# meirbon/rfw-rs

Measured on AMD Instinct MI355X. Metric: Mrays/s (primary+shadow, 1spp), higher is better.
Workload: dtype f32

## Files before the change

rfw-rs_amd/csrc/api_frame.cpp:

```cpp
#include "api_internal.h"

using namespace rfwapi;

namespace rfwapi {
thread_local std::string g_create_error;
}
namespace rfwhip {
static EnvSwitches g_env;
const EnvSwitches& env_switches() { return g_env; }
void read_env_switches()
{
    EnvSwitches e;
    auto set = [](const char* name) { const char* v = getenv(name); return v != nullptr && std::strcmp(v, "0") != 0; };
    e.build_trace = set("RFW_BUILD_TRACE");
    e.no_forest = set("RFW_NO_FOREST");
    e.lbvh_fenced = set("RFW_LBVH_FENCED");
    e.p2p_data_cached = set("RFW_P2P_DATA_CACHED");
    e.p2p_flags_finegrained = set("RFW_P2P_FLAGS_FINEGRAINED");
    if (const char* v = getenv("RFW_PACKET_AUTO_MAX_TRIANGLES")) e.packet_auto_max_triangles = strtoull(v, nullptr, 10);
    if (const char* v = getenv("RFW_SPATIAL_SPLITS")) { e.has_spatial_splits = true; e.spatial_splits = (float)std::max(0.0, atof(v)); }
    if (const char* v = getenv("RFW_PACKET_TRACE")) e.packet_trace = std::max(0, atoi(v));
    static std::mutex mu;
    std::lock_guard<std::mutex> g(mu);
    g_env = e;
// ... 737 lines not shown
        I->release_deform();
        if (I->dn_chain) (void)hipEventDestroy(I->dn_chain);
        I->d_disp_state.release(); I->d_disp_hist.release();
        if (I->disp_chain) (void)hipEventDestroy(I->disp_chain);
        release_overlay(I);
        for (auto& ev : I->ring)
            if (ev) (void)hipEventDestroy(ev);
        if (I->ev_fork) (void)hipEventDestroy(I->ev_fork);
        for (int k = 0; k < kMaxSub; k++) {
            if (I->ev_join[k]) (void)hipEventDestroy(I->ev_join[k]);
            if (I->sub[k]) (void)hipStreamDestroy(I->sub[k]);
        }
        if (I->own_stream) (void)hipStreamDestroy(I->own_stream);
    }
    delete I;
}

const char* rfw_hip_last_error(void* inst)
{
    if (!inst) return g_create_error.c_str();
    return static_cast<Instance*>(inst)->err.c_str();
}


static int render_impl(Instance* I, const rfw_camera_view_3d* views, uint32_t k, bool samples = false, uint32_t mode = RFW_HIP_RENDER_DEFAULT)
{
    if (I->slots.empty()) return do_render(I, views, k, samples, mode);
    Instance* cur = slot_ptr(I, I->cur_slot);
    const bool same_image = (k == 1 || samples) && !I->restart && cur->sample_count > 0 && cur->have_last_view &&
                            std::memcmp(&cur->last_view, views, sizeof(*views)) == 0 && cur->rendered_version == I->scene_version &&
                            cur->render_mode == mode;
    if (!same_image) {
        I->cur_slot = (I->cur_slot + 1) % (uint32_t)(I->slots.size() + 1);
        cur = slot_ptr(I, I->cur_slot);
        cur->sample_count = 0;
    }
    I->restart = false;
    cur->rendered_version = I->scene_version;
    if (cur != I) {
        cur->max_path_length = I->max_path_length; cur->clamp_value = I->clamp_value; cur->flags = I->flags; cur->timing = I->timing;
        for (int c = 0; c < 3; c++) cur->sky[c] = I->sky[c];
        cur->ao_samples = I->ao_samples; cur->ao_radius = I->ao_radius;
        cur->denoise = I->denoise; cur->denoise_colour = I->denoise_colour; cur->denoise_form = I->denoise_form;
    }
    int rc = ensure_slot_tlas(I, cur);
    if (rc == RFW_HIP_OK) rc = do_render(cur, views, k, samples, mode);
    if (rc != RFW_HIP_OK && cur != I && !cur->err.empty()) I->err = cur->err;
    return rc;
}

int rfw_hip_render(void* inst, const rfw_mat4* view_2d, const rfw_camera_view_3d* view, uint32_t mode)
{
    LOCK(inst);
    if (!view) return fail(I, RFW_HIP_E_INVALID, "render: null view");
    CHECK_OVERFLOW(I);
    I->view_2d = view_2d;
    const int rc = render_impl(I, view, 1, false, mode <= (uint32_t)RFW_HIP_RENDER_FILTERED_SSAO ? mode : (uint32_t)RFW_HIP_RENDER_DEFAULT);
    I->view_2d = nullptr;
    return rc;
}

int rfw_hip_render_batch(void* inst, const rfw_camera_view_3d* views, uint32_t count)
{
    LOCK(inst);
    if (!views || count == 0) return fail(I, RFW_HIP_E_INVALID, "render_batch: no views");
    CHECK_OVERFLOW(I);
    if (count == 1) {
        I->sample_count = 0;
        I->restart = true;
    }
    const int rc = render_impl(I, views, count);
    if (rc == RFW_HIP_OK && count == 1) (I->slots.empty() ? I : slot_ptr(I, I->cur_slot))->after_batch = true;
    return rc;
}

int rfw_hip_render_samples(void* inst, const rfw_camera_view_3d* view, uint32_t count)
{
    LOCK(inst);
    if (!view || count == 0) return fail(I, RFW_HIP_E_INVALID, "render_samples: no view / no samples");
    CHECK_OVERFLOW(I);
    if (count > I->max_batch || count > (uint32_t)kMaxBatch) return fail(I, RFW_HIP_E_INVALID, "render_samples: more samples than options.max_batch");
    if (count == 1) return render_impl(I, view, 1);
    rfw_camera_view_3d views[kMaxBatch];
    for (uint32_t f = 0; f < count; f++) views[f] = *view;
    return render_impl(I, views, count, true);
}


int rfw_hip_resize(void* inst, uint32_t w, uint32_t h, double scale)
{
    LOCK(inst);
    if (w == 0 || h == 0) return fail(I, RFW_HIP_E_INVALID, "resize: zero size");
    uint32_t rw = 0, rh = 0;
    if (!render_size_of(w, h, scale, rw, rh))
        return fail(I, RFW_HIP_E_INVALID, "resize: scale must be finite, 0 < scale <= 4, and the render size at most 16384 per axis");
    if (rw != w || rh != h) {
        const Instance* O = scene_of(I);
        if (I->world > 1 || O->comm || O->loop || O->p2p.data || I->external_slab)
            return fail(I, RFW_HIP_E_STATE, "resize: a render scale that changes the frame's size is not available on an instance that exchanges its frame (world > 1, a communicator, the p2p exchange, a slab output)");
    }
    if (scene_of(I)->p2p.data && (rw != I->width || rh != I->height)) return fail(I, RFW_HIP_E_STATE, "resize: disconnect the p2p exchange first (its buffers are sized for the frame)");
    HIP_TRY(I, hipSetDevice(I->device));
    HIP_TRY(I, hipStreamSynchronize(I->stream));
    for (Instance* c : I->slots) {
        const int rc = rfw_hip_resize(c, w, h, scale);
        if (rc != RFW_HIP_OK) return fail(I, rc, c->err);
    }
    I->restart = true;
    I->window_w = w;
    I->window_h = h;
    I->width = rw;
    I->height = rh;
    I->dn_images = 0;
    I->d_dn_ids.release(); I->d_dn_motion.release();
    for (int q = 0; q < 2; q++) { I->d_dn_history_ids[q].release(); I->d_dn_snapshot[q].release(); I->dn_snap_count[q] = 0; }
    I->dn_motion_count = 0;
    I->release_deform();
    I->disp_have_state = false; I->disp_latest = 0;
    I->ov_frame_prims = I->ov_frame_words = 0;
    I->deferred = Instance::Deferred(); I->acc_source = nullptr; I->presented_valid = false;
    const int arc = alloc_paths(I);
    if (arc == RFW_HIP_OK && (scene_of(I)->comm || scene_of(I)->loop)) {
        const size_t n = (size_t)I->capacity * I->max_batch * 3u;
        HIP_TRY(I, I->d_send.ensure(n));
        HIP_TRY(I, I->d_recv.ensure(n * I->world));
    }
    return arc;
}


int rfw_hip_reset_accumulation(void* inst)
{
    LOCK(inst);
    I->sample_count = 0;
    I->restart = true;
    return RFW_HIP_OK;
}

int rfw_hip_set_option(void* inst, const char* key, double value)
{
    LOCK(inst);
    if (!key) return fail(I, RFW_HIP_E_INVALID, "set_option: null key");
    const std::string k(key);
    if (k == "max_path_length") I->max_path_length = std::max<uint32_t>(1, std::min<uint32_t>((uint32_t)value, kMaxBounces));
    else if (k == "clamp_value") I->clamp_value = (float)value;
    else if (k == "nee") I->flags = value != 0.0 ? (I->flags & ~RFW_HIP_FLAG_NO_NEE) : (I->flags | RFW_HIP_FLAG_NO_NEE);
    else if (k == "count_traversal") I->flags = value != 0.0 ? (I->flags | RFW_HIP_FLAG_COUNT_TRAVERSAL) : (I->flags & ~RFW_HIP_FLAG_COUNT_TRAVERSAL);
    else if (k == "shadow_order") {
        I->flags &= ~(kFlagNearFirstDirectional | kFlagFarFirstPositional);
        if ((int)value == 1) I->flags |= kFlagNearFirstDirectional;
        else if ((int)value == 2) I->flags |= kFlagFarFirstPositional;
    }
    else if (k == "packet_trace") {
        I->flags &= ~(kFlagPacketPrimary | kFlagPacketShadow | kFlagPacketShadowFar);
        I->packet_auto = false;
        if ((int)value & 1) I->flags |= kFlagPacketPrimary;
        if ((int)value & 2) I->flags |= kFlagPacketShadow;
        if ((int)value & 4) I->flags |= kFlagPacketShadowFar;
        if (blas_wide_wanted(I, I->n_tris) && !I->d_blas_wide.ptr && I->n_tris) {
            for (auto& kv : I->meshes) kv.second.dirty = true;
            I->meshes_dirty = true;
            I->layout_valid = false;
        }
    }
    else if (k == "single_space") {
        const int v = value != 0.0 ? 1 : 0;
        if (v != I->single_space_opt) {
            I->single_space_opt = v;
            if (v) I->instances_dirty = true;
        }
    }
    else if (k == "shade_group") {
        if ((int)value != 0 && (int)value != 256 && (int)value != 512) return fail(I, RFW_HIP_E_INVALID, "set_option: shade_group is 0, 256 or 512");
        I->shade_group = (int)value;
    }
    else if (k == "tlas_fused") I->tlas_fused = std::max(0, std::min(2, (int)value));
    else if (k == "sample_count") I->sample_count = (uint32_t)value;
    else if (k == "ao_samples" || k == "ao_radius") {
        if (k == "ao_samples") {
            if (!(value >= 1.0 && value <= (double)kAoMaxSamples)) return fail(I, RFW_HIP_E_INVALID, "set_option: ao_samples is 1 ... 8");
            I->ao_samples = (uint32_t)value;
        } else {
            if (!(value >= 0.0) || !std::isfinite(value)) return fail(I, RFW_HIP_E_INVALID, "set_option: ao_radius is >= 0 (0 = automatic)");
            I->ao_radius = (float)value;
        }
        I->sample_count = 0;
        I->restart = true;
    }
    else if (k == "denoise" || k == "denoise_colour") {
        if (k == "denoise") {
            if (!(value >= 0.0 && value <= (double)kDenoiseMaxPasses) || value != std::floor(value)) return fail(I, RFW_HIP_E_INVALID, "set_option: denoise is 0 (off) or 1 ... 5 passes");
            if ((uint32_t)value == I->denoise) return RFW_HIP_OK;
            I->denoise = (uint32_t)value;
        } else {
            if (!(value > 0.0) || !std::isfinite(value) || !((float)value > 0.0f) || !std::isfinite((float)value)) return fail(I, RFW_HIP_E_INVALID, "set_option: denoise_colour is > 0");
            if ((float)value == I->denoise_colour) return RFW_HIP_OK;
            I->denoise_colour = (float)value;
        }
        I->sample_count = 0;
        I->restart = true;
    }
    else if (k == "sample_offset") {
        if (!(value >= 0.0 && value <= 16777216.0) || value != std::floor(value)) return fail(I, RFW_HIP_E_INVALID, "set_option: sample_offset is an integer 0 ... 2^24");
        if ((uint32_t)value == I->sample_offset) return RFW_HIP_OK;
        I->sample_offset = (uint32_t)value;
        I->sample_count = 0;
        I->restart = true;
    }
    else if (k == "denoise_temporal") {
        if (!(value >= 0.0 && value <= (double)kDenoiseMaxHistory) || value != std::floor(value)) return fail(I, RFW_HIP_E_INVALID, "set_option: denoise_temporal is 0 (off) or 1 ... 64 samples");
        if ((uint32_t)value == I->denoise_temporal) return RFW_HIP_OK;
        I->denoise_temporal = (uint32_t)value;
        I->dn_images = 0;
        I->sample_count = 0;
        I->restart = true;
    }
    else if (k == "denoise_motion") {
        if (value != 0.0 && value != 1.0) return fail(I, RFW_HIP_E_INVALID, "set_option: denoise_motion is 0 (off) or 1");
        if ((uint32_t)value == I->denoise_motion) return RFW_HIP_OK;
        I->denoise_motion = (uint32_t)value;
        I->dn_images = 0;
        I->sample_count = 0;
        I->restart = true;
    }
    else if (k == "denoise_deform") {
        if (value != 0.0 && value != 1.0) return fail(I, RFW_HIP_E_INVALID, "set_option: denoise_deform is 0 (off) or 1");
        if ((uint32_t)value == I->denoise_deform) return RFW_HIP_OK;
        I->denoise_deform = (uint32_t)value;
        I->release_deform();
        for (Instance* c : I->slots) c->release_deform();
        I->dn_images = 0;
        I->sample_count = 0;
        I->restart = true;
    }
    else if (k == "denoise_form") {
        if (value != 0.0 && value != 1.0 && value != 2.0) return fail(I, RFW_HIP_E_INVALID, "set_option: denoise_form is 0, 1 or 2");
        I->denoise_form = (uint32_t)value;
    }
    else if (k == "scale_filter") {
        if (value != 0.0 && value != 1.0) return fail(I, RFW_HIP_E_INVALID, "set_option: scale_filter is 0 (nearest) or 1 (bilinear / area)");
        I->scale_filter = (uint32_t)value;
    }
    else if (k == "tonemap" || k == "exposure" || k == "tonemap_white" || k == "auto_exposure" || k == "exposure_key" || k == "exposure_min" || k == "exposure_max" ||
             k == "exposure_low" || k == "exposure_high" || k == "exposure_speed") {
        DisplayParams& d = I->display;
        const float f = (float)value;
        const bool integer = std::isfinite(value) && value == std::floor(value);
        auto within = [&](float lo, float hi) { return std::isfinite(value) && value >= (double)lo && value <= (double)hi && f >= lo && f <= hi; };
        if (k == "tonemap") {
            if (!integer || value < 0.0 || value > 3.0) return fail(I, RFW_HIP_E_INVALID, "set_option: tonemap is 0 (off), 1 (exposure only), 2 (extended Reinhard) or 3 (ACES fit)");
            d.curve = (uint32_t)value;
        } else if (k == "exposure") {
            if (!within(0x1p-20f, 0x1p20f)) return fail(I, RFW_HIP_E_INVALID, "set_option: exposure is 2^-20 ... 2^20");
            d.exposure = f;
        } else if (k == "tonemap_white") {
            if (!std::isfinite(value) || !(value > 0.0) || !(f > 0.0f) || !std::isfinite(f)) return fail(I, RFW_HIP_E_INVALID, "set_option: tonemap_white is finite and > 0");
            d.white = f;
        } else if (k == "auto_exposure") {
            if (value != 0.0 && value != 1.0) return fail(I, RFW_HIP_E_INVALID, "set_option: auto_exposure is 0 or 1");
            d.automatic = (uint32_t)value;
        } else if (k == "exposure_key") {
            if (!within(0x1p-10f, 0x1p10f)) return fail(I, RFW_HIP_E_INVALID, "set_option: exposure_key is 2^-10 ... 2^10");
            d.key = f;
        } else if (k == "exposure_min") {
            if (!within(0x1p-20f, d.exposure_max)) return fail(I, RFW_HIP_E_INVALID, "set_option: exposure_min is 2^-20 ... exposure_max");
            d.exposure_min = f;
        } else if (k == "exposure_max") {
            if (!within(d.exposure_min, 0x1p20f)) return fail(I, RFW_HIP_E_INVALID, "set_option: exposure_max is exposure_min ... 2^20");
            d.exposure_max = f;
        } else if (k == "exposure_low") {
            if (!integer || value < 0.0 || !(value < (double)d.high)) return fail(I, RFW_HIP_E_INVALID, "set_option: exposure_low is an integer percentage, 0 <= low < exposure_high");
            d.low = (uint32_t)value;
        } else if (k == "exposure_high") {
            if (!integer || !(value > (double)d.low) || value > 100.0) return fail(I, RFW_HIP_E_INVALID, "set_option: exposure_high is an integer percentage, exposure_low < high <= 100");
            d.high = (uint32_t)value;
        } else {
            if (!std::isfinite(value) || !(value > 0.0) || value > 1.0 || !(f > 0.0f)) return fail(I, RFW_HIP_E_INVALID, "set_option: exposure_speed is in (0, 1]");
            d.speed = f;
        }
        I->disp_have_state = false;
        I->disp_latest = 0;
    }
    else if (k == "gather_format") {
        if (value < 0 || value > 2) return fail(I, RFW_HIP_E_INVALID, "set_option: gather_format is 0, 1 or 2");
        I->gather_format = (uint32_t)value;
        for (uint32_t q = 0; q <= I->slots.size(); q++) {
            Instance* c = slot_ptr(I, q);
            c->deferred = Instance::Deferred(); c->acc_source = nullptr; c->presented_valid = false;
        }
    }
    else if (k == "present_rank") I->present_rank = (int)value;
    else if (k == "timing") I->timing = value != 0.0;
    else if (k == "sort_extension_rays") I->sort_extension_rays = std::max(0, std::min(2, (int)value));
    else if (k == "texture_array") { I->texture_array = value != 0.0; I->tex_offsets.clear(); }
    else if (k == "spill_rows") {
        I->spill_rows = std::min<uint32_t>((uint32_t)std::max(0.0, value), (uint32_t)kStackSpill);
        clear_overflow(I);
    }
    else if (k == "sky_r") I->sky[0] = (float)value;
    else if (k == "sky_g") I->sky[1] = (float)value;
    else if (k == "sky_b") I->sky[2] = (float)value;
    else if (k == "sah_max_leaf") I->sah_max_leaf = std::max(1, std::min((int)value, kMaxLeafTris));
    else if (k == "sah_trav_cost") I->sah_trav_cost = (float)value;
    else if (k == "spatial_splits") I->split_tau = (float)std::max(0.0, value);
    else if (k == "stream_run") {
        const uint32_t r = (uint32_t)value;
        if (r != 0 && (r > 64 || (r & (r - 1)) != 0)) return fail(I, RFW_HIP_E_INVALID, "set_option: stream_run must be 0 or a power of two up to 64");
        I->stream_run = r;
        I->stream_auto = false;
    } else if (k == "stream_auto") { I->stream_auto = value != 0.0;
    } else if (k == "stream_leaf_gate") I->stream_leaf_gate = (uint32_t)std::max(1.0, std::min(64.0, value));
    else if (k == "stream_refill") I->stream_refill = (uint32_t)std::max(1.0, std::min(64.0, value));
    else if (k == "p2p_timeout_ms") I->p2p.timeout_ticks = (uint64_t)std::max(1.0, value) * 100000ull;
    else if (k == "build_threads") I->build_threads = std::max(1, (int)value);
    else return fail(I, RFW_HIP_E_INVALID, "set_option: unknown key " + k);
    return RFW_HIP_OK;
}

static int materialize_accumulator(Instance* I)
{
    if (scene_of(I)->gather_format != 0 && gathers_tiles(I))
        return fail(I, RFW_HIP_E_STATE, "read_accumulator: with gather_format 1 / 2 only the finished frame travels; the accumulators stay on the ranks that own the tiles");
    { const int rc = ensure_assembled(I); if (rc != RFW_HIP_OK) return rc; }
    const size_t px = (size_t)I->width * I->height * I->max_batch;
    HIP_TRY(I, I->d_frame_acc.ensure(px));
    if (!I->acc_source) {
        HIP_TRY(I, hipMemsetAsync(I->d_frame_acc.ptr, 0, px * sizeof(float4), I->stream));
        return RFW_HIP_OK;
    }
    CameraParams cam = camera_params(I, I->last_view);
    cam.batch = I->acc_source_batch;
    launch_assemble(I->stream, cam, I->acc_source, I->acc_source_rgb, true, I->cap_v, I->d_frame_acc.ptr, 1u);
    HIP_TRY(I, hipGetLastError());
    return RFW_HIP_OK;
}
static int read_frame_impl(void* inst, uint32_t frame, bool accumulator, float* rgba, uint64_t n);
int rfw_hip_read_framebuffer_at(void* inst, uint32_t frame, float* rgba, uint64_t n) { return read_frame_impl(inst, frame, false, rgba, n); }
int rfw_hip_read_accumulator_at(void* inst, uint32_t frame, float* rgba, uint64_t n) { return read_frame_impl(inst, frame, true, rgba, n); }
static int read_frame_impl(void* inst, uint32_t frame, bool accumulator, float* rgba, uint64_t n)
{
    LOCK(inst);
    const uint64_t fpx = accumulator ? (uint64_t)I->width * I->height : (uint64_t)I->window_w * I->window_h;
    if (!rgba || n != fpx * 4) return fail(I, RFW_HIP_E_INVALID, "read_*_at: size mismatch");
    if (frame >= I->max_batch) return fail(I, RFW_HIP_E_INVALID, "read_*_at: frame index beyond options.max_batch");
    if (!I->slots.empty() && I->cur_slot != 0) {
        Instance* c = slot_ptr(I, I->cur_slot);
        const int rc = read_frame_impl(c, frame, accumulator, rgba, n);
        if (rc != RFW_HIP_OK) I->err = c->err;
        return rc;
    }
    HIP_TRY(I, hipSetDevice(I->device));
    if (accumulator) {
        const int rc = materialize_accumulator(I);
        if (rc != RFW_HIP_OK) return rc;
    } else {
        if (scene_of(I)->gather_format == 2 && gathers_tiles(I))
            return fail(I, RFW_HIP_E_STATE, "read_framebuffer: gather_format 2 leaves the PRESENTED frame only: rfw_hip_download_frame(what = 2)");
        const int rc = ensure_assembled(I);
        if (rc != RFW_HIP_OK) return rc;
    }
    const float4* src = (accumulator ? I->d_frame_acc.ptr : window_frame(I)) + (size_t)frame * fpx;
    HIP_TRY(I, hipMemcpyAsync(rgba, src, n * sizeof(float), hipMemcpyDeviceToHost, I->stream));
    HIP_TRY(I, hipStreamSynchronize(I->stream));
    CHECK_OVERFLOW(I);
    return RFW_HIP_OK;
}

void rfw_hip_srgb_steps(float* out255)
{
    if (out255) std::memcpy(out255, srgb_steps(), 255 * sizeof(float));
}
void* rfw_hip_host_alloc(uint64_t bytes)
{
    void* p = nullptr;
    if (bytes == 0 || hipHostMalloc(&p, bytes, hipHostMallocDefault) != hipSuccess) return nullptr;
    return p;
}
void rfw_hip_host_free(void* p)
{
    if (p) (void)hipHostFree(p);
}
int rfw_hip_download_frame(void* inst, uint32_t what, uint32_t frame, float* host_rgba, uint64_t n)
{
    LOCK(inst);
    const uint64_t px = what == 1 ? (uint64_t)I->width * I->height : (uint64_t)I->window_w * I->window_h;
    if (!host_rgba || n != (what == 2 ? px : px * 4)) return fail(I, RFW_HIP_E_INVALID, "download_frame: size mismatch");
    if (what > 2 || frame >= I->max_batch) return fail(I, RFW_HIP_E_INVALID, "download_frame: bad selector");
    Instance* c = I->slots.empty() ? I : slot_ptr(I, I->cur_slot);
    HIP_TRY(I, hipSetDevice(I->device));
    if (!c->download_done) HIP_TRY(I, hipEventCreateWithFlags(&c->download_done, hipEventDisableTiming));
    if (what == 1) {
        const int rc = materialize_accumulator(c);
        if (rc != RFW_HIP_OK) return fail(I, rc, c->err);
    } else {
        const int rc = ensure_assembled(c);
        if (rc != RFW_HIP_OK) return fail(I, rc, c->err);
    }
    const bool sharded_presented = scene_of(c)->gather_format == 2 && gathers_tiles(c);
    if (sharded_presented) {
        if (what != 2) return fail(I, RFW_HIP_E_STATE, "download_frame: gather_format 2 leaves the PRESENTED frame only (what = 2)");
        if (!c->presented_valid) return fail(I, RFW_HIP_E_STATE, "download_frame: no gathered frame yet");
        HIP_TRY(I, hipMemcpyAsync(host_rgba, c->d_present.ptr + (size_t)frame * px, px * sizeof(uint32_t), hipMemcpyDeviceToHost, c->stream));
        HIP_TRY(I, hipEventRecord(c->download_done, c->stream));
        c->download_dst.push_back(host_rgba);
        return RFW_HIP_OK;
    }
    const float4* src = (what == 1 ? c->d_frame_acc.ptr : window_frame(c)) + (size_t)frame * px;
    void* mapped = nullptr;
    hipPointerAttribute_t attr;
    if (hipPointerGetAttributes(&attr, host_rgba) == hipSuccess && attr.type == hipMemoryTypeHost) mapped = attr.devicePointer;
    else (void)hipGetLastError();
    if (what == 2) {
        uint32_t* out = (uint32_t*)mapped;
        if (!out) {
            HIP_TRY(I, c->d_present.ensure(px));
            out = c->d_present.ptr;
        }
        launch_present(c->stream, src, out, px, srgb_steps(), mapped != nullptr);
        HIP_TRY(I, hipGetLastError());
        if (!mapped) HIP_TRY(I, hipMemcpyAsync(host_rgba, c->d_present.ptr, px * sizeof(uint32_t), hipMemcpyDeviceToHost, c->stream));
    } else {
        HIP_TRY(I, hipMemcpyAsync(host_rgba, src, n * sizeof(float), hipMemcpyDeviceToHost, c->stream));
    }
    HIP_TRY(I, hipEventRecord(c->download_done, c->stream));
    c->download_dst.push_back(host_rgba);
    return RFW_HIP_OK;
}
int rfw_hip_wait_download(void* inst, const void* host_ptr)
{
    LOCK(inst);
    HIP_TRY(I, hipSetDevice(I->device));
    for (size_t k = 0; k <= I->slots.size(); k++) {
        Instance* c = slot_ptr(I, (uint32_t)k);
        if (c->download_dst.empty()) continue;
        if (host_ptr && std::find(c->download_dst.begin(), c->download_dst.end(), host_ptr) == c->download_dst.end()) continue;
        HIP_TRY(I, hipEventSynchronize(c->download_done));
        c->download_dst.clear();
    }
    return RFW_HIP_OK;
}
int rfw_hip_wait_downloads(void* inst) { return rfw_hip_wait_download(inst, nullptr); }

int rfw_hip_read_framebuffer(void* inst, float* rgba, uint64_t n) { return read_frame_impl(inst, 0, false, rgba, n); }
int rfw_hip_read_accumulator(void* inst, float* rgba, uint64_t n) { return read_frame_impl(inst, 0, true, rgba, n); }

static void add_frame_timing(Instance* I, int slot, uint32_t nb, bool nee, rfw_hip_frame_stats* out)
{
    hipEvent_t* e0 = ring_events(I, slot, 0);
    auto el = [&](hipEvent_t a, hipEvent_t b) { float ms = 0.0f; (void)hipEventElapsedTime(&ms, a, b); return ms; };
    out->ms_total += el(e0[EV_FRAME0], e0[EV_FRAME1]);
    out->ms_other += el(e0[kEvBlit], e0[kEvBlit + 1]);
    for (uint32_t s = 0; s < I->substreams; s++) {
        hipEvent_t* ev = ring_events(I, slot, s);
        for (uint32_t b = 0; b < nb; b++) {
            const float tr = el(ev[ev_index(b, 0, 0)], ev[ev_index(b, 0, 1)]);
            if (b == 0) out->ms_trace_primary += tr; else out->ms_trace_extend += tr;
            out->ms_shade += el(ev[ev_index(b, 1, 0)], ev[ev_index(b, 1, 1)]);
            if (nee) out->ms_trace_shadow += el(ev[ev_index(b, 2, 0)], ev[ev_index(b, 2, 1)]);
        }
    }
}

int rfw_hip_get_frame_stats(void* inst, rfw_hip_frame_stats* out)
{
    LOCK(inst);
    if (!out) return fail(I, RFW_HIP_E_INVALID, "get_frame_stats: null out");
    if (!I->slots.empty() && I->cur_slot != 0) {
        Instance* c = slot_ptr(I, I->cur_slot);
        const int rc = rfw_hip_get_frame_stats(c, out);
        if (rc != RFW_HIP_OK) I->err = c->err;
        return rc;
    }
    HIP_TRY(I, hipSetDevice(I->device));
    std::memset(out, 0, sizeof(*out));
    HIP_TRY(I, hipStreamSynchronize(I->stream));
    QueueCounters qc[kMaxSub];
    HIP_TRY(I, hipMemcpy(qc, I->d_counters.ptr + (size_t)I->counter_phase * kMaxSub, I->substreams * sizeof(QueueCounters), hipMemcpyDeviceToHost));
    CHECK_OVERFLOW(I);
    const uint32_t nb = I->last_bounces;
    out->primary_rays = nb ? I->local_pixels : 0;
    for (uint32_t s = 0; s < I->substreams; s++) {
        for (uint32_t b = 0; b + 1 < nb; b++) out->extension_rays += qc[s].ext[b];
        if (!(I->flags & RFW_HIP_FLAG_NO_NEE))
            for (uint32_t b = 0; b < nb; b++)
                for (int k = 0; k < kShadowBuckets; k++) out->shadow_rays += qc[s].shadow[b][k];
        for (int k = 0; k < 3; k++) {
            out->nodes_visited[k] += qc[s].trav[k][0];
            out->tris_tested[k] += qc[s].trav[k][1];
            out->instances_entered[k] += qc[s].trav[k][2];
            out->node_test_executions[k] += qc[s].wave_exec[k][0];
            out->tri_test_executions[k] += qc[s].wave_exec[k][1];
            out->uniform_node_test_executions[k] += qc[s].wave_uniform[k];
            out->wave_max_nodes[k] += qc[s].wave_max_nodes[k];
        }
    }
    out->sample_count = I->sample_count;
    out->bounces = nb;
    out->substreams = I->substreams;
    if (I->frame_recorded && nb) add_frame_timing(I, (int)((I->frame_index - 1) % kTimingRing), nb, !(I->flags & RFW_HIP_FLAG_NO_NEE), out);
    return RFW_HIP_OK;
}

int rfw_hip_drain_timing(void* inst, rfw_hip_frame_stats* sum, uint32_t* frames)
{
    LOCK(inst);
    if (!sum || !frames) return fail(I, RFW_HIP_E_INVALID, "drain_timing: null out");
    HIP_TRY(I, hipSetDevice(I->device));
    HIP_TRY(I, hipStreamSynchronize(I->stream));
    std::memset(sum, 0, sizeof(*sum));
    uint32_t n = 0;
    for (uint64_t f = I->drained_index; f < I->frame_index; f++) {
        const int slot = (int)(f % kTimingRing);
        const uint32_t nb = I->ring_bounces[slot];
        if (!nb) continue;
        add_frame_timing(I, slot, nb, I->ring_nee[slot], sum);
        n++;
    }
    sum->substreams = I->substreams;
    I->drained_index = I->frame_index;
    for (Instance* c : I->slots) {
        rfw_hip_frame_stats cs;
        uint32_t cn = 0;
        const int rc = rfw_hip_drain_timing(c, &cs, &cn);
        if (rc != RFW_HIP_OK) return fail(I, rc, c->err);
        sum->ms_total += cs.ms_total; sum->ms_trace_primary += cs.ms_trace_primary; sum->ms_trace_extend += cs.ms_trace_extend;
        sum->ms_trace_shadow += cs.ms_trace_shadow; sum->ms_shade += cs.ms_shade; sum->ms_other += cs.ms_other;
        n += cn;
    }
    *frames = n;
    return RFW_HIP_OK;
}


int rfw_hip_set_stream(void* inst, void* stream)
{
    LOCK(inst);
    if (!I->slots.empty()) return fail(I, RFW_HIP_E_STATE, "set_stream: an instance with frames in flight launches on its slots' own streams");
    HIP_TRY(I, hipSetDevice(I->device));
    HIP_TRY(I, hipStreamSynchronize(I->stream));
    I->stream = stream ? (hipStream_t)stream : I->own_stream;
    return RFW_HIP_OK;
}

int rfw_hip_get_render_size(void* inst, uint32_t* width, uint32_t* height)
{
    LOCK(inst);
    if (!width || !height) return fail(I, RFW_HIP_E_INVALID, "get_render_size: null out");
    *width = I->width;
    *height = I->height;
    return RFW_HIP_OK;
}

void* rfw_hip_get_stream(void* inst)
{
    if (!inst) return nullptr;
    Instance* I = static_cast<Instance*>(inst);
    std::lock_guard<std::mutex> g(I->mu);
    return (void*)I->stream;
}

int rfw_hip_device_synchronize(void* inst)
{
    LOCK(inst);
    HIP_TRY(I, hipSetDevice(I->device));
    HIP_TRY(I, hipStreamSynchronize(I->stream));
    for (Instance* c : I->slots) HIP_TRY(I, hipStreamSynchronize(c->stream));
    return RFW_HIP_OK;
}

}
```

rfw-rs_amd/csrc/api_internal.h:

```cpp
#pragma once
#include <hip/hip_runtime.h>
#include <dlfcn.h>
#include <unistd.h>
#if __has_include(<rccl/rccl.h>)
#include <rccl/rccl.h>
#else
extern "C" {
typedef struct ncclComm* ncclComm_t;
typedef struct { char internal[128]; } ncclUniqueId;
typedef enum { ncclSuccess = 0 } ncclResult_t;
typedef enum { ncclFloat = 7 } ncclDataType_t;
ncclResult_t ncclGetUniqueId(ncclUniqueId* id);
ncclResult_t ncclCommInitRank(ncclComm_t* comm, int nranks, ncclUniqueId id, int rank);
ncclResult_t ncclCommDestroy(ncclComm_t comm);
ncclResult_t ncclAllGather(const void* send, void* recv, size_t count, ncclDataType_t type, ncclComm_t comm, hipStream_t stream);
const char* ncclGetErrorString(ncclResult_t r);
}
#endif

#include <algorithm>
#include <atomic>
#include <chrono>
#include <cmath>
#include <cstring>
#include <map>
#include <mutex>
#include <string>
#include <thread>
#include <vector>

#include "../../include/rfw_hip.h"
#include "bvh_host.h"
#include "env_switches.h"
#include "kernels.h"
#include "lbvh.h"
#include "sah_build.h"
#include "traverse.h"

using namespace rfwhip;

namespace rfwapi {

extern thread_local std::string g_create_error;

struct Rccl {
    void* lib = nullptr;
    decltype(&ncclGetUniqueId) get_unique_id = nullptr;
    decltype(&ncclCommInitRank) comm_init_rank = nullptr;
    decltype(&ncclCommDestroy) comm_destroy = nullptr;
    decltype(&ncclAllGather) all_gather = nullptr;
    decltype(&ncclGetErrorString) error_string = nullptr;
    std::string error;
    bool load()
    {
        if (all_gather) return true;
        for (const char* name : {"librccl.so.1", "librccl.so", "/opt/rocm/lib/librccl.so.1"}) {
            lib = dlopen(name, RTLD_NOW | RTLD_GLOBAL);
            if (lib) break;
        }
        if (!lib) { error = std::string("cannot load librccl: ") + (dlerror() ? dlerror() : "?"); return false; }
        get_unique_id = (decltype(get_unique_id))dlsym(lib, "ncclGetUniqueId");
        comm_init_rank = (decltype(comm_init_rank))dlsym(lib, "ncclCommInitRank");
        comm_destroy = (decltype(comm_destroy))dlsym(lib, "ncclCommDestroy");
        error_string = (decltype(error_string))dlsym(lib, "ncclGetErrorString");
        all_gather = (decltype(all_gather))dlsym(lib, "ncclAllGather");
        if (!get_unique_id || !comm_init_rank || !comm_destroy || !all_gather || !error_string) { error = "librccl lacks a symbol"; all_gather = nullptr; return false; }
        return true;
    }
};
extern Rccl g_rccl;
struct Instance;
int loop_all_gather(Instance* I, hipStream_t s, uint64_t n_words);
void loop_leave(Instance* owner);
extern std::mutex g_rccl_mu;

template <typename T> struct DevBuf {
    T* ptr = nullptr;
    size_t cap = 0;
    hipError_t ensure(size_t n)
    {
        if (n <= cap) return hipSuccess;
        if (ptr) (void)hipFree(ptr);
        ptr = nullptr;
        cap = 0;
        const size_t want = std::max<size_t>(n, 16);
        hipError_t e = hipMalloc((void**)&ptr, want * sizeof(T));
        if (e == hipSuccess) cap = want;
        return e;
    }
    hipError_t grow_keep(size_t n, size_t keep, hipStream_t s)
    {
        if (n <= cap) return hipSuccess;
        const size_t want = std::max<size_t>(n + n / 2, 16);
        T* np = nullptr;
        hipError_t e = hipMalloc((void**)&np, want * sizeof(T));
        if (e != hipSuccess) return e;
        if (ptr && keep) e = hipMemcpyAsync(np, ptr, std::min(keep, cap) * sizeof(T), hipMemcpyDeviceToDevice, s);
        if (e == hipSuccess) e = hipStreamSynchronize(s);
        if (ptr) (void)hipFree(ptr);
        ptr = np;
        cap = want;
        return e;
    }
    void release()
    {
        if (ptr) (void)hipFree(ptr);
        ptr = nullptr;
        cap = 0;
    }
};
struct PinnedRing {
    struct Block { void* p = nullptr; size_t cap = 0; hipEvent_t ev = nullptr; bool pending = false; };
    std::vector<Block> blocks;
    hipError_t upload(void* dst, const void* src, size_t bytes, hipStream_t s)
    {
        if (bytes == 0) return hipSuccess;
        Block* b = nullptr;
        for (Block& c : blocks) {
            if (c.cap < bytes) continue;
            if (c.pending && hipEventQuery(c.ev) == hipSuccess) c.pending = false;
            if (!c.pending) { b = &c; break; }
        }
        if (!b && blocks.size() >= 64) {
            for (Block& c : blocks) {
                if (c.cap < bytes) continue;
                (void)hipEventSynchronize(c.ev);
                c.pending = false;
                b = &c;
                break;
            }
        }
        if (!b) {
            Block n;
            hipError_t e = hipHostMalloc(&n.p, std::max<size_t>(bytes, 64 << 10), hipHostMallocDefault);
            if (e != hipSuccess) return e;
            n.cap = std::max<size_t>(bytes, 64 << 10);
            if ((e = hipEventCreateWithFlags(&n.ev, hipEventDisableTiming)) != hipSuccess) { (void)hipHostFree(n.p); return e; }
            blocks.push_back(n);
            b = &blocks.back();
        }
        std::memcpy(b->p, src, bytes);
        hipError_t e = hipMemcpyAsync(dst, b->p, bytes, hipMemcpyHostToDevice, s);
        if (e == hipSuccess) e = hipEventRecord(b->ev, s);
        b->pending = e == hipSuccess;
        return e;
    }
    void release()
    {
        for (Block& c : blocks) {
            if (c.ev) (void)hipEventDestroy(c.ev);
            if (c.p) (void)hipHostFree(c.p);
        }
        blocks.clear();
    }
};

struct SplitPiece {
    uint32_t index;
    float lo[3], hi[3];
    uint32_t pad;
};
static_assert(sizeof(SplitPiece) == 32, "SplitPiece");
struct MeshHost {
    size_t n_orig = 0, n_refs = 0;
    float split_tau_used = -1.0f;
    std::vector<SplitPiece> pieces;
    std::vector<rfw_rt_triangle> tris;
    std::vector<TriHead> heads;
    bool pinned = false, pin_failed = false;
    void unpin()
    {
        if (!pinned) return;
        (void)hipHostUnregister(tris.data());
        (void)hipHostUnregister(heads.data());
        pinned = false;
    }
    MeshHost() = default;
    MeshHost(const MeshHost&) = delete;
    MeshHost& operator=(const MeshHost&) = delete;
    ~MeshHost() { unpin(); }
    HostBvh4 bvh;
    std::vector<TriPacket> packets;
    std::vector<rfw_joint_data> skin;
    bool dirty = true;
};
struct DerivedMesh {
    uint32_t record = 0;
    uint32_t src_record = 0;
    size_t skin_offset = 0;
    bool topology_built = false;
    uint32_t node_count = 0;
};
struct TexHost {
    uint32_t w = 0, h = 0, mips = 0, format = 0;
    std::vector<uint32_t> texels;
};
struct InstList {
    rfw_aabb local_aabb{};
    std::vector<rfw_mat4> matrices;
    std::vector<int32_t> skin_ids;
};

constexpr int kDefaultPacketTrace = 1;
constexpr uint64_t kPacketAutoMaxTriangles = 12u << 20;
inline uint64_t packet_auto_limit() { const uint64_t e = env_switches().packet_auto_max_triangles; return e ? e : kPacketAutoMaxTriangles; }
enum EvId { EV_FRAME0 = 0, EV_FRAME1, EV_KERNEL_BASE };
constexpr int kMaxBounces = 8;
constexpr int kKernelsPerBounce = 3;
constexpr int kNumEvents = EV_KERNEL_BASE + 2 * (kMaxBounces * kKernelsPerBounce + 1);
constexpr int kTimingRing = 32;
constexpr size_t kSpillMargin = 65536;
constexpr int kMaxSub = 8;

struct Instance {
    std::mutex mu;
    std::string err;
    int device = 0;
    hipStream_t own_stream = nullptr, stream = nullptr;
    uint32_t width = 0, height = 0;
    uint32_t window_w = 0, window_h = 0;
    uint32_t scale_filter = 1;
    uint32_t max_path_length = 3;
    float clamp_value = 10.0f;
    uint32_t rank = 0, world = 1, tile_size = 64;
    bool after_batch = false;
    hipEvent_t download_done = nullptr;
    const void* acc_source = nullptr;
    bool acc_source_rgb = false;
    uint32_t acc_source_batch = 1;
    std::vector<const void*> download_dst;
    uint32_t max_batch = 1;
    uint32_t builder = RFW_HIP_BUILDER_AUTO;
    bool texture_array = true;
    uint32_t flags = 0;
    float sky[3] = {0, 0, 0};
    bool timing = true;
    int build_threads = 8;
    int sah_max_leaf = 8;
    float sah_trav_cost = 1.0f;

    std::map<uint32_t, MeshHost> meshes;
    std::map<uint32_t, InstList> inst_lists;
    std::vector<rfw_device_material> materials;
    std::vector<rfw_area_light> area_lights;
    std::vector<rfw_point_light> point_lights;
    std::vector<rfw_spot_light> spot_lights;
    std::vector<rfw_directional_light> directional_lights;
    std::vector<TexHost> textures;
    std::vector<uint32_t> tex_offsets;
    std::vector<uint32_t> tex_dirty_idx;
    bool tex_layout_dirty = true;
    TexHost skybox;
    std::vector<std::vector<rfw_mat4>> skins;
    std::map<std::pair<uint32_t, int32_t>, DerivedMesh> derived;
    DevBuf<rfw_joint_data> d_skin_data;
    DevBuf<rfw_mat4> d_joints;
    DevBuf<uint32_t> d_bounds_scratch;
    uint32_t raw_node_origin = 0;
    uint32_t max_derived_tris = 0;
    bool meshes_dirty = true, instances_dirty = true, materials_dirty = true, lights_dirty = true, textures_dirty = true;
    bool synchronized = false;

    DevBuf<Node4Q> d_blas_nodes, d_tlas_nodes;
    DevBuf<Node4> d_blas_raw, d_tlas_raw;
    DevBuf<PacketNode> d_blas_wide, d_tlas_wide;
    DevBuf<Node4Q> d_blas_oct, d_tlas_oct;
    DevBuf<Node4Q> d_blas_oct_abs;
    int single_space_opt = 1;
    bool ss_candidate = false;
    std::map<uint32_t, uint32_t> ss_gid_of_mesh;
    uint64_t blas_serial = 0, ss_expanded_serial = ~0ull;
    uint32_t blas_slots_used = 0;
    bool ss_ready = false;
    uint32_t ss_root = 0;
    DevBuf<TriPacket> d_packets;
    DevBuf<rfw_rt_triangle> d_triangles;
    DevBuf<MeshRecord> d_mesh_records;
    DevBuf<rfw_mat4> d_matrices;
    DevBuf<uint32_t> d_mesh_of_instance, d_tlas_prims;
    DevBuf<InstanceXform> d_xforms;
    DevBuf<InstanceNormal> d_normals;
    static constexpr int kTableVersions = 4;
    struct Tables {
        DevBuf<rfw_device_material> materials;
        DevBuf<rfw_area_light> area;
        DevBuf<rfw_point_light> point;
        DevBuf<rfw_spot_light> spot;
        DevBuf<rfw_directional_light> dir;
        size_t n_mat = 0, n_area = 0, n_point = 0, n_spot = 0, n_dir = 0;
    } tables[kTableVersions];
    uint64_t tables_version = 0;
    uint64_t tables_waited = 0, tables_used = 0;
    uint64_t tables_oldest_pending = ~0ull;
    hipStream_t upload_stream = nullptr;
    hipEvent_t tables_ready = nullptr;
    struct Dirty { bool any = false, all = true; std::vector<uint32_t> idx; void clear() { any = false; all = true; idx.clear(); } };
    Dirty mat_dirty, area_dirty, point_dirty, spot_dirty, dir_dirty;
    DevBuf<uint32_t> d_spill;
    DevBuf<uint32_t> d_tex_data;
    DevBuf<TexDesc> d_tex_desc;
    TexDesc skybox_desc{};
    uint32_t n_textures = 0;
    DevBuf<uint8_t> d_blue_noise;
    bool has_blue_noise = false;
    DevBuf<uint32_t> d_valid_gids, d_tlas_order, d_node_count;
    DevBuf<char> d_stage_dev;
    int tlas_fused = 2;
    DevBuf<DevBox> d_inst_boxes, d_mesh_local, d_tri_boxes;
    DevBuf<char> d_lbvh_ws;
    DevBuf<uint32_t> d_blas_order;
    static constexpr int kStages = 2;
    void* stage_buf[kStages] = {};
    size_t stage_cap[kStages] = {};
    hipEvent_t stage_event[kStages] = {};
    bool stage_pending[kStages] = {};
    int stage_next = 0;
    void* stage = nullptr;
    bool tlas_on_device = true, blas_on_device = false, blas_sah_on_device = false;
    DevBuf<char> d_sah_ws;
    DevBuf<uint32_t> d_mesh_node_counts;
    DevBuf<ForestTree> d_forest;
    DevBuf<uint32_t> d_refit_parent, d_refit_nint, d_refit_arrive;
    DevBuf<QueueCounters> d_counters;
    uint32_t counter_phase = 0;
    uint32_t* overflow_host = nullptr;
    uint32_t* overflow_dev = nullptr;
    uint32_t spill_rows = kStackSpill;
    DevBuf<float> d_q_o, d_q_d, d_q_t;
    DevBuf<rfw_hip_hit> d_q_h;
    DevBuf<uint32_t> d_q_depth;
    DevBuf<uint8_t> d_q_r;
    std::vector<MeshRecord> mesh_records;
    std::map<uint32_t, uint32_t> mesh_index;
    std::vector<uint32_t> record_tri_cap;
    std::vector<uint32_t> record_tri_orig;
    DevBuf<SplitPiece> d_split_pieces;
    std::vector<uint32_t> record_piece_off, record_piece_n;
    float split_tau = 8e-5f;
    uint64_t n_split_refs = 0;
    uint32_t tri_end = 0, node_end = 0;
    uint64_t hole_tris = 0;
    bool layout_valid = false;
    bool node_counts_stale = false;
    uint32_t incremental_builds = 0, full_builds = 0, heads_first_builds = 0, tlas_fused_builds = 0;
    bool packet_auto = true;
    PinnedRing pins;
    uint64_t n_instances = 0, n_valid_instances = 0, n_tris = 0, n_blas_nodes = 0, n_tlas_nodes = 0;
    uint64_t n_tris_logical = 0;
    float ms_blas_build = 0, ms_tlas_build = 0, ms_stage_wait = 0;
    float ms_blas_upload = 0, ms_blas_kernels = 0;
    uint64_t blas_upload_bytes = 0, blas_kernel_bytes = 0;
    struct BuildLane { hipStream_t s = nullptr; hipEvent_t done = nullptr; DevBuf<char> ws; DevBuf<DevBox> boxes; };
    static constexpr int kBuildLanes = 8;
    BuildLane lanes[kBuildLanes];
    hipEvent_t ev_build[3] = {nullptr, nullptr, nullptr};
    DevBuf<TriHead> d_heads;
    hipStream_t records_stream = nullptr;
    hipEvent_t ev_heads = nullptr, ev_records = nullptr;
    bool records_pending = false;
    bool records_timed = false;
    bool build_events_pending = false;

    DevBuf<float4> d_ray_o[2], d_ray_d[2], d_thr[2], d_sh_o, d_sh_d, d_sh_e, d_acc_slab, d_frame_acc, d_frame_out, d_frame_win;
    DevBuf<uint32_t> d_present;
    DevBuf<uint4> d_hit[2];
    DevBuf<uint32_t> d_sort_keys[2], d_sort_vals[2];
    DevBuf<char> d_sort_ws;
    int shade_group = 0;
    int sort_extension_rays = 2;
    void* external_slab = nullptr;
    ncclComm_t comm = nullptr;
    DevBuf<float> d_send, d_recv;
    uint32_t gather_format = 0;
    int present_rank = -1;
    struct Deferred { const void* gathered = nullptr; uint32_t k = 0, samples = 1; } deferred;
    bool presented_valid = false;
    hipEvent_t comm_chain = nullptr;
    bool comm_chain_pending = false;
    struct LoopHub* loop = nullptr;
    uint32_t loop_seq = 0;
    hipEvent_t loop_sent = nullptr;
    struct P2P {
        bool connected = false;
        uint32_t* data = nullptr;
        uint32_t* flags = nullptr;
        size_t slot_words = 0;
        uint32_t n_slots = 0;
        std::vector<uint32_t*> peer_data, peer_flags;
        std::vector<uint8_t> opened;
        uint64_t timeout_ticks = 500000000ull;
    } p2p;
    uint32_t slot_index = 0;
    uint32_t stream_leaf_gate = 16;
    bool stream_auto = true;
    uint32_t stream_run = 8, stream_refill = 12;
    uint32_t p2p_seq = 0;
    bool frame_elsewhere = false;
    uint32_t tiles_x = 0, tiles_y = 0, local_tiles = 0, capacity = 0;
    uint64_t local_pixels = 0;
    uint32_t sample_count = 0;
    bool have_last_view = false;
    rfw_camera_view_3d last_view{};
    uint32_t render_mode = 0;
    uint32_t ao_samples = 4;
    float ao_radius = 0.0f;
    float ao_auto_radius = 0.0f;
    uint64_t ao_auto_version = 0;
    uint32_t ao_rounds = 0;
    DevBuf<float4> d_ao_guide;
    uint32_t denoise = 0;
    float denoise_colour = kDenoiseDefaultColour;
    uint32_t denoise_form = 0;
    DevBuf<float4> d_dn_guide, d_dn_plane[2];
    uint32_t sample_offset = 0;
    uint32_t image_offset = 0;
    uint32_t denoise_temporal = 0;
    DevBuf<float4> d_dn_history[2];
    float dn_view[2][12] = {};
    uint32_t dn_images = 0, dn_latest = 0;
    uint32_t dn_image = 0;
    hipEvent_t dn_chain = nullptr;
    bool dn_chain_pending = false;
    uint32_t denoise_motion = 0;
    DevBuf<uint32_t> d_dn_ids;
    DevBuf<uint32_t> d_dn_history_ids[2];
    DevBuf<char> d_dn_snapshot[2], d_dn_motion;
    uint32_t dn_snap_count[2] = {}, dn_motion_count = 0;
    uint32_t denoise_deform = 0;
    DevBuf<uint2> d_dn_tris;
    DevBuf<float4> d_dn_pose[2];
    DevBuf<uint4> d_dn_refs[2], d_dn_copies;
    std::vector<uint4> dn_copies;
    uint32_t dn_pose_tris[2] = {};
    bool dn_deform_latest = false;
    void release_deform()
    {
        d_dn_tris.release(); d_dn_copies.release();
        for (int q = 0; q < 2; q++) { d_dn_pose[q].release(); d_dn_refs[q].release(); dn_pose_tris[q] = 0; }
        dn_copies.clear();
        dn_deform_latest = false;
    }
    DisplayParams display;
    DevBuf<uint32_t> d_disp_state;
    bool disp_have_state = false;
    uint32_t disp_latest = 0;
    float disp_manual = 1.0f;
    hipEvent_t disp_chain = nullptr;
    bool disp_chain_pending = false;
    DevBuf<uint32_t> d_disp_hist;
    struct Mesh2D { std::vector<rfw_vertex_2d> vertices; int32_t tex = -1; std::vector<rfw_mat4> matrices; };
    std::map<uint32_t, Mesh2D> meshes_2d;
    bool ov_dirty = false;
    struct OvVersion {
        DevBuf<rfw_vertex_2d> vertices;
        DevBuf<OvDraw> draws;
        uint32_t n_draws = 0, n_prims = 0;
    } ov[kTableVersions];
    uint64_t ov_version = 0;
    uint64_t ov_waited = 0;
    uint64_t ov_oldest_pending = ~0ull;
    hipEvent_t ov_ready = nullptr;
    const rfw_mat4* view_2d = nullptr;
    DevBuf<OvPrim> d_ov_prims;
    DevBuf<OvTap> d_ov_tap;
    DevBuf<uint64_t> d_ov_words;
    uint32_t ov_frame_prims = 0, ov_frame_words = 0;
    const rfw_mat4* d_forward = nullptr;
    std::vector<hipEvent_t> ring;
    hipEvent_t* events = nullptr;
    uint32_t substreams = 1;
    hipStream_t sub[kMaxSub] = {};
    hipEvent_t ev_fork = nullptr, ev_join[kMaxSub] = {};
    uint32_t local_tiles_v = 0, cap_v = 0;
    uint64_t frame_index = 0, drained_index = 0;
    uint32_t ring_bounces[kTimingRing] = {};
    bool ring_nee[kTimingRing] = {};
    uint32_t last_bounces = 0;
    bool frame_recorded = false;
    bool last_count_flag = false;

    Instance* scene = nullptr;
    std::vector<Instance*> slots;
    uint32_t cur_slot = 0;
    uint64_t scene_version = 1;
    uint64_t rendered_version = 0;
    uint64_t waited_version = 0;
    uint64_t instances_version = 1;
    uint64_t tlas_version = 0;
    bool restart = false;
    hipEvent_t scene_ready = nullptr;
    hipEvent_t frame_done = nullptr;
};

inline bool scaled(const Instance* I) { return I->window_w != I->width || I->window_h != I->height; }
inline float4* window_frame(Instance* I) { return scaled(I) ? I->d_frame_win.ptr : I->d_frame_out.ptr; }
inline bool render_size_of(const uint32_t w, const uint32_t h, const double scale, uint32_t& rw, uint32_t& rh)
{
    if (!std::isfinite(scale) || !(scale > 0.0) || !(scale <= 4.0)) return false;
    const double x = (double)w * scale, y = (double)h * scale;
    if (x >= 16385.0 || y >= 16385.0) return false;
    rw = std::max(1u, (uint32_t)x);
    rh = std::max(1u, (uint32_t)y);
    return true;
}
#define REFUSE_SCALED(inst, what)                                                                                                                   \
    do {                                                                                                                                            \
        if (scaled(inst)) return fail(inst, RFW_HIP_E_STATE, what ": not available where the render size differs from the window size (a scaled frame is not exchanged)"); \
    } while (0)
constexpr uint32_t kSingleSpaceMaxInstances = 256;
constexpr uint32_t kGraftSlots = 2 * kSingleSpaceMaxInstances;
inline uint32_t graft_reserve(const Instance* I) { return (uint32_t)(1 + I->slots.size()) * kGraftSlots; }
inline Instance* scene_of(Instance* I) { return I->scene ? I->scene : I; }
inline const Instance* scene_of(const Instance* I) { return I->scene ? I->scene : I; }
void p2p_release(Instance* I);
inline Instance* slot_ptr(Instance* I, uint32_t k) { return k == 0 ? I : I->slots[k - 1]; }
inline bool per_slot_tlas(const Instance* S) { return !S->slots.empty() && S->derived.empty(); }
inline Instance* tlas_of(Instance* I) { Instance* S = scene_of(I); return per_slot_tlas(S) ? I : S; }

#define HIP_TRY(inst, expr)                                                                     \
    do {                                                                                        \
        hipError_t e_ = (expr);                                                                 \
        if (e_ != hipSuccess) {                                                                 \
            (inst)->err = std::string(#expr) + ": " + hipGetErrorString(e_);                    \
            return RFW_HIP_E_DEVICE;                                                            \
        }                                                                                       \
    } while (0)

inline int fail(Instance* I, int code, const std::string& msg)
{
    I->err = msg;
    return code;
}

inline bool overflow_seen(const Instance* I)
{
    if (I->overflow_host && *(volatile const uint32_t*)I->overflow_host) return true;
    for (const Instance* c : I->slots)
        if (c->overflow_host && *(volatile const uint32_t*)c->overflow_host) return true;
    return false;
}
inline void clear_overflow(Instance* I)
{
// ... 54 lines not shown
```

rfw-rs_amd/csrc/api_scene.cpp:

```cpp
#include "api_internal.h"
#if defined(__SSE2__)
#include <emmintrin.h>
#endif

using namespace rfwapi;

static_assert(sizeof(rfw_hip_scene_stats) == 96 && offsetof(rfw_hip_scene_stats, single_space) == 92, "rfw_hip_scene_stats is a public POD (rfw-rs_amd/pod.py mirrors it): new fields need a new RFW_HIP_ABI_VERSION");

namespace rfwapi {
hipError_t follow_copies(DevBuf<PacketNode>& wide, DevBuf<Node4Q>& oct, const DevBuf<Node4Q>& nodes, size_t keep, hipStream_t s, bool want_wide)
{
    const size_t want = nodes.cap * kPacketNodeCopies;
    if (!want_wide && wide.ptr) wide.release();
    if (oct.cap == want && (wide.cap == want || !want_wide)) return hipSuccess;
    const bool oct_kept = oct.cap == want;
    wide.release();
    if (!oct_kept) oct.release();
    if (want == 0) return hipSuccess;
    hipError_t e = hipSuccess;
    if (want_wide) {
        e = hipMalloc((void**)&wide.ptr, want * sizeof(PacketNode));
        if (e != hipSuccess) { wide.ptr = nullptr; return e; }
        wide.cap = want;
    }
    if (!oct_kept) {
        e = hipMalloc((void**)&oct.ptr, want * sizeof(Node4Q));
        if (e != hipSuccess) { oct.ptr = nullptr; return e; }
        oct.cap = want;
    }
    OctantCopies oc;
    oc.wide = wide.ptr; oc.quant = oct.ptr; oc.stride = (uint32_t)nodes.cap;
    launch_expand_nodes(s, nodes.ptr, oc, 0u, (uint32_t)std::min(keep, nodes.cap));
    return hipGetLastError();
}
inline OctantCopies copies_of(const DevBuf<PacketNode>& wide, const DevBuf<Node4Q>& oct)
{
    OctantCopies oc;
    oc.wide = wide.ptr; oc.quant = oct.ptr; oc.stride = (uint32_t)(oct.cap / kPacketNodeCopies);
    return oc;
}
bool blas_wide_wanted(const Instance* I, uint64_t n_prims)
{
    if (!(I->flags & (kFlagPacketPrimary | kFlagPacketShadow | kFlagPacketShadowFar))) return false;
    return !(I->packet_auto && n_prims > packet_auto_limit());
}

inline void pad_box(PrimBox& b)
{
    for (int a = 0; a < 3; a++) {
        const float m = std::max(std::fabs(b.lo[a]), std::fabs(b.hi[a]));
        const float e = 1e-4f + 4e-6f * m;
        b.lo[a] -= e;
        b.hi[a] += e;
    }
}

void build_mesh(Instance* I, MeshHost& m)
{
    const size_t n = m.n_refs;
    std::vector<PrimBox> boxes(n);
    for (size_t i = 0; i < n; i++) {
        const rfw_rt_triangle& t = m.tris[i];
        const float* v[3] = {&t.vertex0.x, &t.vertex1.x, &t.vertex2.x};
        for (int a = 0; a < 3; a++) {
            boxes[i].lo[a] = std::min(v[0][a], std::min(v[1][a], v[2][a]));
            boxes[i].hi[a] = std::max(v[0][a], std::max(v[1][a], v[2][a]));
        }
        pad_box(boxes[i]);
    }
    for (const SplitPiece& sp : m.pieces) {
        for (int a = 0; a < 3; a++) { boxes[sp.index].lo[a] = sp.lo[a]; boxes[sp.index].hi[a] = sp.hi[a]; }
        pad_box(boxes[sp.index]);
    }
    build_bvh4_host(boxes, I->sah_max_leaf, I->build_threads, m.bvh, I->sah_trav_cost);
    m.packets.resize(n);
    for (size_t k = 0; k < n; k++) {
        const uint32_t id = m.bvh.prim_order[k];
        const rfw_rt_triangle& t = m.tris[id];
        TriPacket p;
        p.v0x = t.vertex0.x; p.v0y = t.vertex0.y; p.v0z = t.vertex0.z;
        p.tri_id = id;
        if (id >= m.n_orig) std::memcpy(&p.tri_id, reinterpret_cast<const float*>(&t) + 15, 4);
        p.e1x = t.vertex1.x - t.vertex0.x; p.e1y = t.vertex1.y - t.vertex0.y; p.e1z = t.vertex1.z - t.vertex0.z;
        p.e2x = t.vertex2.x - t.vertex0.x; p.e2y = t.vertex2.y - t.vertex0.y; p.e2z = t.vertex2.z - t.vertex0.z;
        p.inv_gn2 = 1.0f / (t.normal.x * t.normal.x + t.normal.y * t.normal.y + t.normal.z * t.normal.z);
        p.pad = 0.0f;
        m.packets[k] = p;
    }
    m.dirty = false;
}

int ensure_stage(Instance* I, size_t bytes)
{
    const int k = I->stage_next;
    I->stage = I->stage_buf[k];
    if (bytes <= I->stage_cap[k]) return RFW_HIP_OK;
    if (I->stage_buf[k]) (void)hipHostFree(I->stage_buf[k]);
    I->stage_buf[k] = nullptr;
    I->stage = nullptr;
    I->stage_cap[k] = 0;
    const size_t want = std::max<size_t>(bytes * 2, 1 << 20);
    HIP_TRY(I, hipHostMalloc(&I->stage_buf[k], want, hipHostMallocDefault));
    I->stage_cap[k] = want;
    I->stage = I->stage_buf[k];
    return RFW_HIP_OK;
}

int ensure_lbvh_ws(Instance* I, uint32_t n)
{
    const size_t need = lbvh_workspace_bytes(n);
    HIP_TRY(I, I->d_lbvh_ws.ensure(need));
    return RFW_HIP_OK;
}

std::map<std::pair<uint32_t, int32_t>, DerivedMesh> wanted_derived(const Instance* I)
{
    std::map<std::pair<uint32_t, int32_t>, DerivedMesh> out;
    for (const auto& kv : I->inst_lists) {
        const auto mit = I->meshes.find(kv.first);
        if (mit == I->meshes.end() || mit->second.skin.empty()) continue;
        for (size_t s = 0; s < kv.second.matrices.size(); s++) {
            const int32_t sk = s < kv.second.skin_ids.size() ? kv.second.skin_ids[s] : -1;
            if (sk < 0 || (size_t)sk >= I->skins.size() || I->skins[sk].empty() || is_zero_matrix(kv.second.matrices[s])) continue;
            out[std::make_pair(kv.first, sk)];
        }
    }
    return out;
}

int layout_derived(Instance* I, uint32_t& tri_total, uint32_t& node_total)
{
    const uint32_t static_nodes = node_total;
    I->derived = wanted_derived(I);
    I->max_derived_tris = 0;
    std::vector<rfw_joint_data> skin_all;
    std::map<uint32_t, size_t> skin_off;
    for (auto& kv : I->derived) {
        DerivedMesh& d = kv.second;
        d.src_record = I->mesh_index[kv.first.first];
        const MeshHost& src = I->meshes[kv.first.first];
        auto so = skin_off.find(kv.first.first);
        if (so == skin_off.end()) {
            so = skin_off.emplace(kv.first.first, skin_all.size()).first;
            skin_all.insert(skin_all.end(), src.skin.begin(), src.skin.end());
        }
        d.skin_offset = so->second;
        MeshRecord r;
        std::memset(&r, 0, sizeof(r));
        r.tri_base = tri_total;
        r.tri_count = (uint32_t)src.n_orig;
        r.node_base = node_total;
        r.node_count = std::max<uint32_t>(r.tri_count, 1u);
        tri_total += r.tri_count;
        node_total += r.node_count;
        d.record = (uint32_t)I->mesh_records.size();
        I->mesh_records.push_back(r);
        I->record_tri_orig.resize(I->mesh_records.size(), 0u);
        I->record_tri_orig.back() = r.tri_count;
        I->max_derived_tris = std::max(I->max_derived_tris, r.tri_count);
    }
    if (I->derived.empty()) return RFW_HIP_OK;
    if (!I->blas_on_device) {
        I->raw_node_origin = static_nodes;
        HIP_TRY(I, I->d_blas_raw.ensure(node_total - static_nodes));
    }
    HIP_TRY(I, I->d_blas_order.ensure(tri_total));
    HIP_TRY(I, I->d_tri_boxes.ensure(I->max_derived_tris));
    HIP_TRY(I, I->d_bounds_scratch.ensure(8));
    return upload(I, I->d_skin_data, skin_all.data(), skin_all.size());
}

uint64_t build_pass_bytes(uint64_t n)
{
    uint32_t levels = 0;
    for (uint64_t v = n / 512u; v > 0; v >>= 1) levels++;
    return n * (208u + 116u * levels + 40u + 228u) + (n / 4u) * 320u;
}

struct RecordSource { uint32_t q; const MeshHost* mesh; };
struct BuildPlan {
    bool from_heads;
    bool quantise_now;
};

int upload_split_pieces(Instance* I, const std::vector<RecordSource>& build)
{
    I->record_piece_off.assign(I->mesh_records.size(), 0u);
    I->record_piece_n.assign(I->mesh_records.size(), 0u);
    std::vector<SplitPiece> all;
    for (const RecordSource& b : build) {
        if (b.mesh->pieces.empty()) continue;
        I->record_piece_off[b.q] = (uint32_t)all.size();
        I->record_piece_n[b.q] = (uint32_t)b.mesh->pieces.size();
        all.insert(all.end(), b.mesh->pieces.begin(), b.mesh->pieces.end());
    }
    if (all.empty()) return RFW_HIP_OK;
    HIP_TRY(I, I->d_split_pieces.ensure(all.size()));
    HIP_TRY(I, I->pins.upload(I->d_split_pieces.ptr, all.data(), all.size() * sizeof(SplitPiece), I->stream));
    return RFW_HIP_OK;
}
inline void patch_boxes(Instance* I, hipStream_t s, uint32_t q, DevBox* boxes)
{
    if (q < I->record_piece_n.size() && I->record_piece_n[q]) launch_patch_boxes(s, I->d_split_pieces.ptr + I->record_piece_off[q], I->record_piece_n[q], boxes);
}
inline void resolve_duplicates(Instance* I, hipStream_t s, uint32_t q)
{
    const MeshRecord& r = I->mesh_records[q];
    if (q < I->record_tri_orig.size() && I->record_tri_orig[q] < r.tri_count)
        launch_resolve_duplicates(s, I->d_packets.ptr + r.tri_base, r.tri_count, r.tri_base, I->record_tri_orig[q], I->d_triangles.ptr + r.tri_base);
}
inline void record_boxes(Instance* I, hipStream_t s, uint32_t q, bool from_heads, DevBox* out)
{
    const MeshRecord& r = I->mesh_records[q];
    if (from_heads) launch_triangle_boxes(s, I->d_heads.ptr + r.tri_base, r.tri_count, out);
    else launch_triangle_boxes(s, I->d_triangles.ptr + r.tri_base, r.tri_count, out);
    patch_boxes(I, s, q, out);
}
inline void record_packets(Instance* I, hipStream_t s, uint32_t q)
{
    const MeshRecord& r = I->mesh_records[q];
    launch_make_packets(s, I->d_triangles.ptr + r.tri_base, I->d_blas_order.ptr + r.tri_base, r.tri_count, r.tri_base, I->d_packets.ptr + r.tri_base);
    resolve_duplicates(I, s, q);
}
inline void record_finish(Instance* I, hipStream_t s, uint32_t q, const BuildPlan& plan)
{
    const MeshRecord& r = I->mesh_records[q];
    if (!plan.from_heads) record_packets(I, s, q);
    if (plan.quantise_now)
        launch_quantize_nodes(s, I->d_blas_raw.ptr + r.node_base, I->d_blas_nodes.ptr + r.node_base, copies_of(I->d_blas_wide, I->d_blas_oct), r.node_base, std::max(r.tri_count, 1u), I->d_mesh_node_counts.ptr + q);
}

int build_tree(Instance* I, hipStream_t s, bool sah, const DevBox* boxes, uint32_t n, DevBuf<char>& sah_ws, const DevBuf<char>& lbvh_ws, Node4* raw, uint32_t* order, uint32_t* count)
{
    if (sah) {
        HIP_TRY(I, sah_ws.ensure(sah_workspace_bytes(n)));
        const hipError_t se = sah_build(s, boxes, n, sah_ws.ptr, sah_ws.cap, raw, order, count, I->sah_max_leaf, I->sah_trav_cost);
        if (se != hipErrorInvalidValue) { HIP_TRY(I, se); return RFW_HIP_OK; }
    }
    HIP_TRY(I, lbvh_build(s, boxes, n, lbvh_ws.ptr, lbvh_ws.cap, raw, order, count));
    return RFW_HIP_OK;
}

int build_mesh_device(Instance* I, uint32_t q, const BuildPlan& plan)
{
    const MeshRecord& r = I->mesh_records[q];
    if (r.tri_count == 0) return RFW_HIP_OK;
    record_boxes(I, I->stream, q, plan.from_heads, I->d_tri_boxes.ptr);
    const int rc = build_tree(I, I->stream, I->blas_sah_on_device, I->d_tri_boxes.ptr, r.tri_count, I->d_sah_ws, I->d_lbvh_ws, I->d_blas_raw.ptr + r.node_base,
                              I->d_blas_order.ptr + r.tri_base, I->d_mesh_node_counts.ptr + q);
    if (rc == RFW_HIP_OK) record_finish(I, I->stream, q, plan);
    return rc;
}

int build_meshes(Instance* I, const std::vector<RecordSource>& build, const BuildPlan plan)
{
    constexpr uint32_t kSmallMesh = 131072;
    std::vector<uint32_t> small, large;
    for (const RecordSource& b : build) (I->blas_sah_on_device && I->mesh_records[b.q].tri_count && I->mesh_records[b.q].tri_count <= kSmallMesh ? small : large).push_back(b.q);
    if (small.size() < 2) { large.clear(); for (const RecordSource& b : build) large.push_back(b.q); small.clear(); }
    int rc = RFW_HIP_OK;
    const int n_lanes = (int)std::min<size_t>(Instance::kBuildLanes, small.size());
    std::vector<std::thread> workers;
    std::vector<hipError_t> lane_err((size_t)std::max(n_lanes, 1), hipSuccess);
    std::vector<uint8_t> redo(I->mesh_records.size(), 0);
    std::atomic<size_t> next{0};
    if (n_lanes) {
        uint32_t max_n = 0;
        for (const uint32_t q : small) max_n = std::max(max_n, I->mesh_records[q].tri_count);
        hipEvent_t start = I->ev_build[1];
        for (int k = 0; k < n_lanes; k++) {
            Instance::BuildLane& L = I->lanes[k];
            if (!L.s) HIP_TRY(I, hipStreamCreateWithFlags(&L.s, hipStreamNonBlocking));
            if (!L.done) HIP_TRY(I, hipEventCreateWithFlags(&L.done, hipEventDisableTiming));
            HIP_TRY(I, L.ws.ensure(sah_workspace_bytes(max_n)));
            HIP_TRY(I, L.boxes.ensure(max_n));
            HIP_TRY(I, hipStreamWaitEvent(L.s, start, 0));
        }
        for (int k = 0; k < n_lanes; k++)
            workers.emplace_back([I, k, &small, &next, &lane_err, &redo, plan] {
                Instance::BuildLane& L = I->lanes[k];
                if (hipSetDevice(I->device) != hipSuccess) { lane_err[k] = hipErrorInvalidDevice; return; }
                for (size_t i = next.fetch_add(1); i < small.size(); i = next.fetch_add(1)) {
                    const uint32_t q = small[i];
                    const MeshRecord& r = I->mesh_records[q];
                    record_boxes(I, L.s, q, plan.from_heads, L.boxes.ptr);
                    const hipError_t e = sah_build(L.s, L.boxes.ptr, r.tri_count, L.ws.ptr, L.ws.cap, I->d_blas_raw.ptr + r.node_base, I->d_blas_order.ptr + r.tri_base,
                                                   I->d_mesh_node_counts.ptr + q, I->sah_max_leaf, I->sah_trav_cost);
                    if (e == hipErrorInvalidValue) { redo[q] = 1; continue; }
                    if (e != hipSuccess) { lane_err[k] = e; return; }
                    record_finish(I, L.s, q, plan);
                }
                (void)hipEventRecord(L.done, L.s);
            });
    }
    for (const uint32_t q : large)
        if (rc == RFW_HIP_OK) rc = build_mesh_device(I, q, plan);
    for (auto& t : workers) t.join();
    for (int k = 0; k < n_lanes; k++) {
        if (lane_err[k] != hipSuccess && rc == RFW_HIP_OK) rc = fail(I, RFW_HIP_E_DEVICE, std::string("build lane: ") + hipGetErrorString(lane_err[k]));
        (void)hipStreamWaitEvent(I->stream, I->lanes[k].done, 0);
    }
    if (rc != RFW_HIP_OK) return rc;
    for (const uint32_t q : small)
        if (redo[q] && (rc = build_mesh_device(I, q, plan))) return rc;
    return RFW_HIP_OK;
}

void assign_logical_ids(Instance* I)
{
    uint32_t logical = 0;
    for (auto& kv : I->meshes) {
        const auto it = I->mesh_index.find(kv.first);
        if (it == I->mesh_index.end()) continue;
        I->mesh_records[it->second].tri_logical = logical;
        logical += I->record_tri_orig[it->second];
    }
    for (auto& kv : I->derived) {
        I->mesh_records[kv.second.record].tri_logical = logical;
        logical += I->mesh_records[kv.second.record].tri_count;
    }
    I->n_tris_logical = logical;
}

int upload_heads_first(Instance* I, const std::vector<RecordSource>& send, size_t heads_cap)
{
    HIP_TRY(I, I->d_heads.ensure(heads_cap));
    if (!I->records_stream) HIP_TRY(I, hipStreamCreateWithFlags(&I->records_stream, hipStreamNonBlocking));
    if (!I->ev_heads) HIP_TRY(I, hipEventCreate(&I->ev_heads));
    if (!I->ev_records) HIP_TRY(I, hipEventCreate(&I->ev_records));
    for (int pass = 0; pass < 2; pass++)
        for (const RecordSource& b : send) {
            const MeshRecord& r = I->mesh_records[b.q];
            if (!r.tri_count || (int)b.mesh->pinned != pass) continue;
            const size_t bytes = (size_t)r.tri_count * sizeof(TriHead);
            if (b.mesh->pinned) HIP_TRY(I, hipMemcpyAsync(I->d_heads.ptr + r.tri_base, b.mesh->heads.data(), bytes, hipMemcpyHostToDevice, I->stream));
            else HIP_TRY(I, I->pins.upload(I->d_heads.ptr + r.tri_base, b.mesh->heads.data(), bytes, I->stream));
        }
    HIP_TRY(I, hipEventRecord(I->ev_heads, I->stream));
    HIP_TRY(I, hipStreamWaitEvent(I->records_stream, I->ev_heads, 0));
    for (int pass = 0; pass < 2; pass++)
        for (const RecordSource& b : send) {
            const MeshRecord& r = I->mesh_records[b.q];
            if (!r.tri_count || (int)b.mesh->pinned != pass) continue;
            const size_t bytes = (size_t)r.tri_count * sizeof(rfw_rt_triangle);
            if (b.mesh->pinned) HIP_TRY(I, hipMemcpyAsync(I->d_triangles.ptr + r.tri_base, b.mesh->tris.data(), bytes, hipMemcpyHostToDevice, I->records_stream));
            else HIP_TRY(I, I->pins.upload(I->d_triangles.ptr + r.tri_base, b.mesh->tris.data(), bytes, I->records_stream));
        }
    HIP_TRY(I, hipEventRecord(I->ev_records, I->records_stream));
    I->records_pending = true;
    I->records_timed = true;
    I->heads_first_builds++;
    return RFW_HIP_OK;
}

void trim_build_scratch(Instance* I, size_t limit)
{
    if (I->d_sah_ws.cap > limit) I->d_sah_ws.release();
    for (auto& L : I->lanes)
        if (L.ws.cap > limit) { L.ws.release(); L.boxes.release(); }
}

struct BuildTrace {
    const bool on = env_switches().build_trace;
    const std::chrono::steady_clock::time_point t_start = std::chrono::steady_clock::now();
    void operator()(const char* what) const { if (on) fprintf(stderr, "[build] %-28s %7.3f ms\n", what, std::chrono::duration<float, std::milli>(std::chrono::steady_clock::now() - t_start).count()); }
};
struct FullLayout {
    std::vector<RecordSource> statics;
    uint32_t static_tris = 0, static_nodes = 0, tri_total = 0, node_total = 0, max_n = 0;
};

int layout_records(Instance* I, FullLayout& L)
{
    I->mesh_records.clear();
    I->mesh_index.clear();
    I->record_tri_cap.clear();
    I->record_tri_orig.clear();
    for (auto& kv : I->meshes) {
        MeshRecord r;
        std::memset(&r, 0, sizeof(r));
        r.tri_base = L.tri_total;
        r.tri_count = (uint32_t)kv.second.n_refs;
        I->record_tri_orig.push_back((uint32_t)kv.second.n_orig);
        r.node_base = L.node_total;
        r.node_count = std::max<uint32_t>(r.tri_count, 1u);
        L.tri_total += r.tri_count;
        L.node_total += r.node_count;
        L.max_n = std::max(L.max_n, r.tri_count);
        L.statics.push_back(RecordSource{(uint32_t)I->mesh_records.size(), &kv.second});
        I->mesh_index[kv.first] = (uint32_t)I->mesh_records.size();
        I->mesh_records.push_back(r);
        I->record_tri_cap.push_back(r.tri_count);
        kv.second.dirty = false;
    }
    L.static_nodes = L.node_total;
    L.static_tris = L.tri_total;
    I->raw_node_origin = 0;
    if (const int rc = layout_derived(I, L.tri_total, L.node_total)) return rc;
    assign_logical_ids(I);
    HIP_TRY(I, I->d_triangles.ensure(L.tri_total));
    HIP_TRY(I, I->d_packets.ensure(L.tri_total));
    HIP_TRY(I, I->d_blas_nodes.ensure((size_t)L.node_total + graft_reserve(I)));
    I->blas_slots_used = L.node_total;
    HIP_TRY(I, follow_copies(I->d_blas_wide, I->d_blas_oct, I->d_blas_nodes, 0, I->stream, blas_wide_wanted(I, L.tri_total)));
    HIP_TRY(I, I->d_blas_raw.ensure(L.node_total));
    HIP_TRY(I, I->d_blas_order.ensure(L.tri_total));
    return RFW_HIP_OK;
}

int build_static_trees(Instance* I, const FullLayout& L, bool from_heads, const BuildTrace& trace)
{
    const size_t n_static = L.statics.size();
    HIP_TRY(I, I->d_tri_boxes.ensure(std::max(L.max_n, I->max_derived_tris)));
    if (const int rc = ensure_lbvh_ws(I, L.max_n)) return rc;
    HIP_TRY(I, I->d_mesh_node_counts.ensure(std::max<size_t>(n_static, 1)));
    HIP_TRY(I, hipMemsetAsync(I->d_mesh_node_counts.ptr, 0, std::max<size_t>(n_static, 1) * 4, I->stream));
    HIP_TRY(I, hipEventRecord(I->ev_build[1], I->stream));
    constexpr size_t forest_min = 4;
    if (I->blas_sah_on_device && n_static >= forest_min && L.static_tris > 0 && !env_switches().no_forest) {
        std::vector<ForestTree> trees(n_static);
        for (size_t q = 0; q < n_static; q++) trees[q] = ForestTree{I->mesh_records[q].tri_base, I->mesh_records[q].tri_count, I->mesh_records[q].node_base, 0u};
        HIP_TRY(I, I->d_forest.ensure(n_static));
        HIP_TRY(I, I->pins.upload(I->d_forest.ptr, trees.data(), n_static * sizeof(ForestTree), I->stream));
        HIP_TRY(I, I->d_tri_boxes.ensure(std::max(L.static_tris, I->max_derived_tris)));
        HIP_TRY(I, I->d_sah_ws.ensure(sah_forest_workspace_bytes(L.static_tris, (uint32_t)n_static)));
        if (from_heads) launch_triangle_boxes(I->stream, I->d_heads.ptr, L.static_tris, I->d_tri_boxes.ptr);
        else launch_triangle_boxes(I->stream, I->d_triangles.ptr, L.static_tris, I->d_tri_boxes.ptr);
        for (size_t q = 0; q < n_static; q++) patch_boxes(I, I->stream, (uint32_t)q, I->d_tri_boxes.ptr + I->mesh_records[q].tri_base);
        const hipError_t fe = sah_build_forest(I->stream, I->d_tri_boxes.ptr, L.static_tris, I->d_forest.ptr, (uint32_t)n_static, L.max_n, I->d_sah_ws.ptr, I->d_sah_ws.cap,
                                               I->d_blas_raw.ptr, I->d_blas_order.ptr, I->d_mesh_node_counts.ptr, I->sah_max_leaf, I->sah_trav_cost);
        if (fe == hipSuccess) {
            if (from_heads) HIP_TRY(I, hipStreamWaitEvent(I->stream, I->ev_records, 0));
            launch_make_packets(I->stream, I->d_triangles.ptr, I->d_blas_order.ptr, L.static_tris, 0u, I->d_packets.ptr);
            for (size_t q = 0; q < n_static; q++) resolve_duplicates(I, I->stream, (uint32_t)q);
            launch_forest_relative_order(I->stream, I->d_blas_order.ptr, L.static_tris, I->d_forest.ptr, (uint32_t)n_static);
            return RFW_HIP_OK;
        }
        if (fe != hipErrorInvalidValue) HIP_TRY(I, fe);
    }
    const int rc = build_meshes(I, L.statics, BuildPlan{from_heads, false});
    trace("trees queued");
    if (from_heads) {
        HIP_TRY(I, hipStreamWaitEvent(I->stream, I->ev_records, 0));
        if (rc == RFW_HIP_OK)
            for (size_t q = 0; q < n_static; q++)
                if (I->mesh_records[q].tri_count) record_packets(I, I->stream, (uint32_t)q);
    }
    return rc;
}

int finish_full_build(Instance* I, const FullLayout& L, const BuildTrace& trace)
{
    const size_t n_static = L.statics.size();
    if (const int rc = upload(I, I->d_mesh_records, I->mesh_records.data(), I->mesh_records.size())) return rc;
    launch_quantize_regions(I->stream, I->d_blas_raw.ptr, I->d_blas_nodes.ptr, copies_of(I->d_blas_wide, I->d_blas_oct), L.static_nodes, I->d_mesh_records.ptr,
                            I->d_mesh_node_counts.ptr, (uint32_t)n_static);
    HIP_TRY(I, hipGetLastError());
    I->n_tris = L.tri_total;
    I->n_split_refs = 0;
    for (size_t q = 0; q < n_static; q++) I->n_split_refs += I->mesh_records[q].tri_count - I->record_tri_orig[q];
    HIP_TRY(I, hipEventRecord(I->ev_build[2], I->stream));
    trace("all queued");
    HIP_TRY(I, hipStreamSynchronize(I->stream));
    I->records_pending = false;
    trace("device done");
    if (trace.on && I->records_timed) {
        float a = 0, b = 0, c = 0;
        (void)hipEventElapsedTime(&c, I->ev_build[0], I->ev_heads);
        fprintf(stderr, "[build] by events: heads arrived %.3f ms\n", c);
        (void)hipEventElapsedTime(&a, I->ev_build[0], I->ev_records);
        (void)hipEventElapsedTime(&b, I->ev_build[0], I->ev_build[2]);
        fprintf(stderr, "[build] by events: records arrived %.3f ms, build done %.3f ms after the start\n", a, b);
    }
    I->build_events_pending = true;
    I->blas_upload_bytes = (uint64_t)L.static_tris * sizeof(rfw_rt_triangle);
    I->blas_kernel_bytes = 0;
    for (size_t q = 0; q < n_static; q++) I->blas_kernel_bytes += build_pass_bytes(I->mesh_records[q].tri_count);
    std::vector<uint32_t> counts(n_static, 0u);
    if (n_static) HIP_TRY(I, hipMemcpy(counts.data(), I->d_mesh_node_counts.ptr, n_static * 4, hipMemcpyDeviceToHost));
    I->n_blas_nodes = L.node_total - L.static_nodes;
    for (uint32_t c : counts) I->n_blas_nodes += c;
    I->node_counts_stale = false;
    trim_build_scratch(I, size_t(1) << 30);
    I->tri_end = L.static_tris;
    I->node_end = L.static_nodes;
    I->hole_tris = 0;
    I->layout_valid = I->derived.empty();
    I->full_builds++;
    return RFW_HIP_OK;
}

int upload_static_meshes(Instance* I, const FullLayout& L, const BuildTrace& trace, bool& heads_first)
{
    for (auto& ev : I->ev_build)
        if (!ev) HIP_TRY(I, hipEventCreate(&ev));
    HIP_TRY(I, hipEventRecord(I->ev_build[0], I->stream));
    if (const int rc = upload_split_pieces(I, L.statics)) return rc;
    bool any_pinned = false;
    for (const RecordSource& b : L.statics) any_pinned = any_pinned || b.mesh->pinned;
    heads_first = any_pinned && L.static_tris > 0;
    I->records_timed = false;
    if (heads_first) {
        if (const int rc = upload_heads_first(I, L.statics, L.static_tris)) return rc;
        trace("uploads queued");
    } else {
        for (const RecordSource& b : L.statics)
            if (const MeshRecord& r = I->mesh_records[b.q]; r.tri_count)
                HIP_TRY(I, hipMemcpyAsync(I->d_triangles.ptr + r.tri_base, b.mesh->tris.data(), (size_t)r.tri_count * sizeof(rfw_rt_triangle), hipMemcpyHostToDevice, I->stream));
    }
    return RFW_HIP_OK;
}

int build_blas_device_full(Instance* I)
{
    const BuildTrace trace{};
    FullLayout L;
    bool heads_first = false;
    int rc;
    if ((rc = layout_records(I, L))) return rc;
    if ((rc = upload_static_meshes(I, L, trace, heads_first))) return rc;
    if ((rc = build_static_trees(I, L, heads_first, trace))) return rc;
    return finish_full_build(I, L, trace);
}

int build_blas_device_incremental(Instance* I)
{
    I->records_timed = false;
    for (auto it = I->mesh_index.begin(); it != I->mesh_index.end();) {
        if (I->meshes.find(it->first) == I->meshes.end()) {
            I->hole_tris += I->record_tri_cap[it->second];
            I->mesh_records[it->second].tri_count = 0;
            it = I->mesh_index.erase(it);
        } else ++it;
    }
    std::vector<RecordSource> todo;
    uint32_t max_n = 0;
    for (auto& kv : I->meshes) {
        MeshHost& m = kv.second;
        if (!m.dirty) continue;
        const uint32_t n = (uint32_t)m.n_refs;
        uint32_t q;
        const auto it = I->mesh_index.find(kv.first);
        if (it != I->mesh_index.end() && n <= I->record_tri_cap[it->second]) {
            q = it->second;
        } else {
            if (it != I->mesh_index.end()) {
                q = it->second;
                I->hole_tris += I->record_tri_cap[q];
            } else {
                q = (uint32_t)I->mesh_records.size();
                MeshRecord r;
                std::memset(&r, 0, sizeof(r));
                I->mesh_records.push_back(r);
                I->record_tri_cap.push_back(0);
                I->record_tri_orig.push_back(0);
                I->mesh_index[kv.first] = q;
            }
            if ((uint64_t)I->tri_end + n > kLeafFirstMask || (uint64_t)I->node_end + std::max(n, 1u) > 0x7fffffffu) return 1;
            I->mesh_records[q].tri_base = I->tri_end;
            I->mesh_records[q].node_base = I->node_end;
            I->record_tri_cap[q] = n;
            I->tri_end += n;
            I->node_end += std::max(n, 1u);
        }
        I->mesh_records[q].tri_count = n;
        I->record_tri_orig[q] = (uint32_t)m.n_orig;
        I->mesh_records[q].node_count = std::max(I->record_tri_cap[q], 1u);
        todo.push_back(RecordSource{q, &m});
        max_n = std::max(max_n, n);
        m.dirty = false;
    }
    if (I->hole_tris > std::max<uint64_t>(I->tri_end / 2, 1u << 16)) return 1;
    assign_logical_ids(I);
    HIP_TRY(I, I->d_triangles.grow_keep(I->tri_end, I->d_triangles.cap, I->stream));
    HIP_TRY(I, I->d_packets.grow_keep(I->tri_end, I->d_packets.cap, I->stream));
    HIP_TRY(I, I->d_blas_order.grow_keep(I->tri_end, I->d_blas_order.cap, I->stream));
    {
        const size_t nodes_before = I->d_blas_nodes.cap;
        HIP_TRY(I, I->d_blas_nodes.grow_keep((size_t)I->node_end + graft_reserve(I), I->d_blas_nodes.cap, I->stream));
        I->blas_slots_used = I->node_end;
        HIP_TRY(I, follow_copies(I->d_blas_wide, I->d_blas_oct, I->d_blas_nodes, nodes_before, I->stream, blas_wide_wanted(I, I->tri_end)));
    }
    HIP_TRY(I, I->d_blas_raw.grow_keep(I->node_end, 0, I->stream));
    HIP_TRY(I, I->d_mesh_node_counts.grow_keep(std::max<size_t>(I->mesh_records.size(), 1), I->d_mesh_node_counts.cap, I->stream));
    HIP_TRY(I, I->d_mesh_records.grow_keep(std::max<size_t>(I->mesh_records.size(), 1), 0, I->stream));
    HIP_TRY(I, I->d_tri_boxes.ensure(std::max(max_n, 1u)));
    int rc;
    if ((rc = ensure_lbvh_ws(I, max_n))) return rc;
    for (auto& ev : I->ev_build)
        if (!ev) HIP_TRY(I, hipEventCreate(&ev));
    HIP_TRY(I, hipEventRecord(I->ev_build[0], I->stream));
    if ((rc = upload_split_pieces(I, todo))) return rc;
    I->blas_upload_bytes = I->blas_kernel_bytes = 0;
    for (const RecordSource& b : todo) {
        I->blas_upload_bytes += (uint64_t)I->mesh_records[b.q].tri_count * sizeof(rfw_rt_triangle);
        I->blas_kernel_bytes += build_pass_bytes(I->mesh_records[b.q].tri_count);
    }
    const bool heads_first = todo.size() == 1 && I->mesh_records[todo[0].q].tri_count * sizeof(rfw_rt_triangle) >= (size_t(1) << 20) && todo[0].mesh->pinned;
    if (heads_first && (rc = upload_heads_first(I, todo, I->tri_end))) return rc;
    for (const RecordSource& b : todo) {
        if (heads_first) break;
        const MeshRecord& r = I->mesh_records[b.q];
        const size_t bytes = (size_t)r.tri_count * sizeof(rfw_rt_triangle);
        if (bytes <= (8u << 20)) HIP_TRY(I, I->pins.upload(I->d_triangles.ptr + r.tri_base, b.mesh->tris.data(), bytes, I->stream));
        else {
            HIP_TRY(I, hipMemcpyAsync(I->d_triangles.ptr + r.tri_base, b.mesh->tris.data(), bytes, hipMemcpyHostToDevice, I->stream));
            HIP_TRY(I, hipStreamSynchronize(I->stream));
        }
    }
    HIP_TRY(I, hipEventRecord(I->ev_build[1], I->stream));
    if ((rc = build_meshes(I, todo, BuildPlan{heads_first, true}))) return rc;
    if (heads_first) {
        HIP_TRY(I, hipStreamWaitEvent(I->stream, I->ev_records, 0));
        record_packets(I, I->stream, todo[0].q);
    }
    HIP_TRY(I, hipEventRecord(I->ev_build[2], I->stream));
    I->build_events_pending = true;
    HIP_TRY(I, hipGetLastError());
    HIP_TRY(I, I->pins.upload(I->d_mesh_records.ptr, I->mesh_records.data(), I->mesh_records.size() * sizeof(MeshRecord), I->stream));
    I->n_tris = I->n_split_refs = 0;
    for (auto& kv : I->mesh_index) {
        I->n_tris += I->mesh_records[kv.second].tri_count;
        I->n_split_refs += I->mesh_records[kv.second].tri_count - I->record_tri_orig[kv.second];
    }
    I->node_counts_stale = true;
    I->incremental_builds++;
    return RFW_HIP_OK;
}

int build_blas_device(Instance* I)
{
    bool any_dirty = false, removed = false, all_dirty = !I->meshes.empty();
    for (auto& kv : I->meshes) { any_dirty = any_dirty || kv.second.dirty; all_dirty = all_dirty && kv.second.dirty; }
    for (auto& kv : I->mesh_index) removed = removed || I->meshes.find(kv.first) == I->meshes.end();
    if (I->layout_valid && I->derived.empty() && wanted_derived(I).empty() && (any_dirty || removed) && !(all_dirty && I->meshes.size() >= 2)) {
        const int rc = build_blas_device_incremental(I);
        trim_build_scratch(I, 64u << 20);
        if (rc < 0) {
            I->layout_valid = false;
            for (auto& kv : I->meshes) kv.second.dirty = true;
            I->meshes_dirty = true;
        }
        if (rc <= 0) return rc;
        for (auto& kv : I->meshes) kv.second.dirty = true;
    }
    return build_blas_device_full(I);
}

int build_blas_host(Instance* I)
{
    for (auto& kv : I->meshes)
        if (kv.second.dirty) build_mesh(I, kv.second);
    I->mesh_records.clear();
    I->mesh_index.clear();
    I->record_tri_orig.clear();
    I->n_split_refs = 0;
    I->layout_valid = false;
    std::vector<Node4> nodes;
    std::vector<TriPacket> packets;
    std::vector<rfw_rt_triangle> tris;
    for (auto& kv : I->meshes) {
        MeshHost& m = kv.second;
        MeshRecord r;
        std::memset(&r, 0, sizeof(r));
        r.node_base = (uint32_t)nodes.size();
        r.node_count = (uint32_t)m.bvh.nodes.size();
        r.tri_base = (uint32_t)tris.size();
        r.tri_count = (uint32_t)m.n_refs;
        I->mesh_index[kv.first] = (uint32_t)I->mesh_records.size();
        I->mesh_records.push_back(r);
        I->record_tri_orig.push_back((uint32_t)m.n_orig);
        I->n_split_refs += m.n_refs - m.n_orig;
        nodes.insert(nodes.end(), m.bvh.nodes.begin(), m.bvh.nodes.end());
        const size_t p0 = packets.size();
        packets.insert(packets.end(), m.packets.begin(), m.packets.end());
        for (size_t k = p0; k < packets.size(); k++) packets[k].tri_id += r.tri_base;
        tris.insert(tris.end(), m.tris.begin(), m.tris.begin() + (ptrdiff_t)m.n_refs);
    }
    uint32_t tri_total = (uint32_t)tris.size(), node_total = (uint32_t)nodes.size();
    int rc;
    if ((rc = layout_derived(I, tri_total, node_total))) return rc;
    assign_logical_ids(I);
    I->n_tris = tri_total;
    I->n_blas_nodes = node_total;
    HIP_TRY(I, I->d_blas_nodes.ensure((size_t)node_total + graft_reserve(I)));
    I->blas_slots_used = node_total;
    HIP_TRY(I, follow_copies(I->d_blas_wide, I->d_blas_oct, I->d_blas_nodes, 0, I->stream, blas_wide_wanted(I, tri_total)));
    HIP_TRY(I, I->d_packets.ensure(tri_total));
    HIP_TRY(I, I->d_triangles.ensure(tri_total));
    std::vector<Node4Q> qnodes(nodes.size());
    for (size_t k = 0; k < nodes.size(); k++) qnodes[k] = quantize_node(nodes[k]);
    if ((rc = upload(I, I->d_blas_nodes, qnodes.data(), qnodes.size()))) return rc;
    launch_expand_nodes(I->stream, I->d_blas_nodes.ptr, copies_of(I->d_blas_wide, I->d_blas_oct), 0u, (uint32_t)qnodes.size());
    if ((rc = upload(I, I->d_packets, packets.data(), packets.size()))) return rc;
    if ((rc = upload(I, I->d_triangles, tris.data(), tris.size()))) return rc;
    if ((rc = upload(I, I->d_mesh_records, I->mesh_records.data(), I->mesh_records.size()))) return rc;
    HIP_TRY(I, hipStreamSynchronize(I->stream));
    return RFW_HIP_OK;
}

bool single_space_candidate(const Instance* I, std::map<uint32_t, uint32_t>& gid_of_mesh)
{
    gid_of_mesh.clear();
    if (I->single_space_opt == 0 || !I->tlas_on_device || !wanted_derived(I).empty()) return false;
    static const rfw_mat4 identity = {{1.0f, 0.0f, 0.0f, 0.0f, 0.0f, 1.0f, 0.0f, 0.0f, 0.0f, 0.0f, 1.0f, 0.0f, 0.0f, 0.0f, 0.0f, 1.0f}};
    uint32_t gid = 0;
    uint64_t tris = 0;
    for (const auto& kv : I->inst_lists) {
        const auto mit = I->meshes.find(kv.first);
        const bool mesh_ok = mit != I->meshes.end() && mit->second.n_refs > 0;
        for (size_t k = 0; k < kv.second.matrices.size(); k++, gid++) {
            if (!mesh_ok || is_zero_matrix(kv.second.matrices[k])) continue;
            if (std::memcmp(&kv.second.matrices[k], &identity, sizeof(rfw_mat4)) != 0) return false;
            if (!gid_of_mesh.emplace(kv.first, gid).second) return false;
            tris += mit->second.n_refs;
        }
    }
    return !gid_of_mesh.empty() && gid_of_mesh.size() <= kSingleSpaceMaxInstances && tris <= kLeafFirstMask;
}
bool single_space_layout_fits(const Instance* I, const std::map<uint32_t, uint32_t>& gid_of_mesh)
{
    const uint64_t stride = I->d_blas_oct.cap / kPacketNodeCopies;
    if ((uint64_t)I->blas_slots_used + graft_reserve(I) > stride) return false;
    for (const auto& kv : gid_of_mesh) {
        const auto it = I->mesh_index.find(kv.first);
        if (it == I->mesh_index.end()) return false;
        const MeshRecord& r = I->mesh_records[it->second];
        if ((uint64_t)r.node_base + r.node_count > I->blas_slots_used || (uint64_t)r.tri_base + r.tri_count > kLeafFirstMask) return false;
    }
    return true;
}
int prepare_single_space(Instance* I, const std::map<uint32_t, uint32_t>& gid_of_mesh)
{
// ... 1159 lines not shown
```

rfw-rs_amd/csrc/bvh_host.cpp:

```cpp
#include "bvh_host.h"

#include <algorithm>
#include <atomic>
#include <cmath>
#include <future>

namespace rfwhip {
namespace {

constexpr int kBinCount = 16;

struct B3 {
    float lo[3], hi[3];
    void reset()
    {
        for (int a = 0; a < 3; a++) { lo[a] = INFINITY; hi[a] = -INFINITY; }
    }
    void grow(const float* l, const float* h)
    {
        for (int a = 0; a < 3; a++) { lo[a] = std::min(lo[a], l[a]); hi[a] = std::max(hi[a], h[a]); }
    }
    void grow_pt(const float* p)
    {
        for (int a = 0; a < 3; a++) { lo[a] = std::min(lo[a], p[a]); hi[a] = std::max(hi[a], p[a]); }
    }
    float half_area() const
    {
        const float ex = hi[0] - lo[0], ey = hi[1] - lo[1], ez = hi[2] - lo[2];
        if (!(ex >= 0.0f) || !(ey >= 0.0f) || !(ez >= 0.0f)) return 0.0f;
        return ex * ey + ey * ez + ez * ex;
    }
};

struct Node2 {
    B3 box;
    uint32_t left = 0, right = 0;
    uint32_t first = 0, count = 0;
};

struct Builder2 {
    const std::vector<PrimBox>& boxes;
    std::vector<float> cent;
    std::vector<uint32_t> order;
    std::vector<Node2> nodes;
    std::atomic<uint32_t> next_node{1};
    int max_leaf;
    int max_par_depth;
    float trav_cost = 1.0f;

    Builder2(const std::vector<PrimBox>& b, int ml, int threads) : boxes(b), max_leaf(ml)
    {
        const size_t n = b.size();
        cent.resize(3 * n);
        order.resize(n);
        for (size_t i = 0; i < n; i++) {
            order[i] = (uint32_t)i;
            for (int a = 0; a < 3; a++) cent[3 * i + a] = 0.5f * (b[i].lo[a] + b[i].hi[a]);
        }
        nodes.resize(n ? 2 * n : 1);
        max_par_depth = 0;
        while ((1 << max_par_depth) < threads * 4) max_par_depth++;
    }

    void build(uint32_t ni, uint32_t first, uint32_t count, int depth)
    {
        Node2& node = nodes[ni];
        node.box.reset();
        B3 cb;
        cb.reset();
        for (uint32_t i = 0; i < count; i++) {
            const uint32_t p = order[first + i];
            node.box.grow(boxes[p].lo, boxes[p].hi);
            cb.grow_pt(&cent[3 * p]);
        }
        node.first = first;
        node.count = count;
        if (count <= 1) return;

        float best_cost = INFINITY;
        int best_axis = -1, best_plane = -1;
        for (int a = 0; a < 3; a++) {
            const float lo = cb.lo[a], hi = cb.hi[a];
            if (!(hi > lo)) continue;
            const float scale = (float)kBinCount / (hi - lo);
            B3 bin_box[kBinCount];
            uint32_t bin_cnt[kBinCount];
            for (int b = 0; b < kBinCount; b++) { bin_box[b].reset(); bin_cnt[b] = 0; }
            for (uint32_t i = 0; i < count; i++) {
                const uint32_t p = order[first + i];
                int b = (int)((cent[3 * p + a] - lo) * scale);
                b = std::min(std::max(b, 0), kBinCount - 1);
                bin_cnt[b]++;
                bin_box[b].grow(boxes[p].lo, boxes[p].hi);
            }
            float right_area[kBinCount];
            uint32_t right_cnt[kBinCount];
            B3 acc;
            acc.reset();
            uint32_t c = 0;
            for (int b = kBinCount - 1; b > 0; b--) {
                acc.grow(bin_box[b].lo, bin_box[b].hi);
                c += bin_cnt[b];
                right_area[b] = acc.half_area();
                right_cnt[b] = c;
            }
            acc.reset();
            c = 0;
            for (int b = 0; b < kBinCount - 1; b++) {
                acc.grow(bin_box[b].lo, bin_box[b].hi);
                c += bin_cnt[b];
                if (c == 0 || right_cnt[b + 1] == 0) continue;
                const float cost = (float)c * acc.half_area() + (float)right_cnt[b + 1] * right_area[b + 1];
                if (cost < best_cost) { best_cost = cost; best_axis = a; best_plane = b; }
            }
        }
        uint32_t mid = 0;
        const float leaf_cost = (float)count * node.box.half_area();
        if (best_axis >= 0 && (best_cost + trav_cost * node.box.half_area() < leaf_cost || (int)count > max_leaf)) {
            const float lo = cb.lo[best_axis], hi = cb.hi[best_axis];
            const float scale = (float)kBinCount / (hi - lo);
            uint32_t* begin = &order[first];
            uint32_t* m = std::partition(begin, begin + count, [&](uint32_t p) {
                int b = (int)((cent[3 * p + best_axis] - lo) * scale);
                b = std::min(std::max(b, 0), kBinCount - 1);
                return b <= best_plane;
            });
            mid = (uint32_t)(m - begin);
        } else if ((int)count > max_leaf) {
            mid = count / 2;
        }
        if (mid == 0 || mid >= count) return;
        const uint32_t li = next_node.fetch_add(2);
        node.left = li;
        node.right = li + 1;
        node.count = 0;
        if (depth < max_par_depth && count > 8192) {
            auto fut = std::async(std::launch::async, [=]() { build(li, first, mid, depth + 1); });
            build(li + 1, first + mid, count - mid, depth + 1);
            fut.get();
        } else {
            build(li, first, mid, depth + 1);
            build(li + 1, first + mid, count - mid, depth + 1);
        }
    }
};

inline void set_child(Node4& n, int slot, const B3& b, uint32_t ref)
{
    n.lox[slot] = b.lo[0]; n.loy[slot] = b.lo[1]; n.loz[slot] = b.lo[2];
    n.hix[slot] = b.hi[0]; n.hiy[slot] = b.hi[1]; n.hiz[slot] = b.hi[2];
    n.child[slot] = ref;
}
inline Node4 empty_node4()
{
    Node4 n;
    for (int i = 0; i < 4; i++) {
        n.lox[i] = n.loy[i] = n.loz[i] = INFINITY;
        n.hix[i] = n.hiy[i] = n.hiz[i] = -INFINITY;
        n.child[i] = kInvalidRef;
        n.pad[i] = 0;
    }
    return n;
}

}

void build_bvh4_host(const std::vector<PrimBox>& boxes, int max_leaf, int threads, HostBvh4& out, float trav_cost)
{
    out.nodes.clear();
    out.prim_order.clear();
    out.nodes.push_back(empty_node4());
    const uint32_t n = (uint32_t)boxes.size();
    if (n == 0) return;
    max_leaf = std::min(std::max(max_leaf, 1), kMaxLeafTris);
    Builder2 b2(boxes, max_leaf, std::max(threads, 1));
    b2.trav_cost = trav_cost;
    b2.build(0, 0, n, 0);
    out.prim_order = b2.order;
    const std::vector<Node2>& n2 = b2.nodes;

    if (n2[0].count > 0) {
        set_child(out.nodes[0], 0, n2[0].box, make_leaf(n2[0].first, n2[0].count));
        return;
    }
    struct Work { uint32_t n4, n2; };
    std::vector<Work> stack;
    stack.push_back({0u, 0u});
    while (!stack.empty()) {
        const Work w = stack.back();
        stack.pop_back();
        uint32_t kids[4] = {n2[w.n2].left, n2[w.n2].right, 0, 0};
        int nk = 2;
        while (nk < 4) {
            int best = -1;
            float best_area = -1.0f;
            for (int i = 0; i < nk; i++) {
                if (n2[kids[i]].count > 0) continue;
                const float a = n2[kids[i]].box.half_area();
                if (a > best_area) { best_area = a; best = i; }
            }
            if (best < 0) break;
            const uint32_t k = kids[best];
            kids[best] = n2[k].left;
            kids[nk++] = n2[k].right;
        }
        for (int i = 0; i < nk; i++) {
            const Node2& k = n2[kids[i]];
            if (k.count > 0) {
                set_child(out.nodes[w.n4], i, k.box, make_leaf(k.first, k.count));
            } else {
                const uint32_t id = (uint32_t)out.nodes.size();
                out.nodes.push_back(empty_node4());
                set_child(out.nodes[w.n4], i, k.box, id);
                stack.push_back({id, kids[i]});
            }
        }
    }
}

uint64_t validate_bvh4(const HostBvh4& bvh, const std::vector<PrimBox>& boxes)
{
    uint64_t errors = 0;
    std::vector<uint32_t> seen(boxes.size(), 0);
    if (bvh.nodes.empty()) return boxes.empty() ? 0 : 1;
    struct W { uint32_t node; float lo[3], hi[3]; };
    std::vector<W> st;
    st.push_back({0u, {-INFINITY, -INFINITY, -INFINITY}, {INFINITY, INFINITY, INFINITY}});
    while (!st.empty()) {
        const W w = st.back();
        st.pop_back();
        const Node4& n = bvh.nodes[w.node];
        for (int i = 0; i < 4; i++) {
            if (n.child[i] == kInvalidRef) continue;
            const float lo[3] = {n.lox[i], n.loy[i], n.loz[i]}, hi[3] = {n.hix[i], n.hiy[i], n.hiz[i]};
            for (int a = 0; a < 3; a++)
                if (lo[a] < w.lo[a] || hi[a] > w.hi[a]) errors++;
            if (n.child[i] & kLeafBit) {
                const uint32_t first = n.child[i] & kLeafFirstMask, count = ((n.child[i] >> 27) & 15u) + 1u;
                for (uint32_t k = 0; k < count; k++) {
                    if (first + k >= bvh.prim_order.size()) { errors++; continue; }
                    const uint32_t p = bvh.prim_order[first + k];
                    seen[p]++;
                    for (int a = 0; a < 3; a++)
                        if (boxes[p].lo[a] < lo[a] || boxes[p].hi[a] > hi[a]) errors++;
                }
            } else {
                W c{n.child[i], {lo[0], lo[1], lo[2]}, {hi[0], hi[1], hi[2]}};
                st.push_back(c);
            }
        }
    }
    for (uint32_t s : seen)
        if (s != 1) errors++;
    return errors;
}

}
```

rfw-rs_amd/csrc/bvh_host.h:

```cpp
#pragma once
#include <cstdint>
#include <vector>

#include "device_types.h"

namespace rfwhip {

struct PrimBox {
    float lo[3], hi[3];
};

struct HostBvh4 {
    std::vector<Node4> nodes;
    std::vector<uint32_t> prim_order;
};

void build_bvh4_host(const std::vector<PrimBox>& boxes, int max_leaf, int threads, HostBvh4& out, float trav_cost = 1.0f);

uint64_t validate_bvh4(const HostBvh4& bvh, const std::vector<PrimBox>& boxes);

}
```

rfw-rs_amd/csrc/sah_build.h:

```cpp
#pragma once
#include <hip/hip_runtime.h>

#include <cstddef>
#include <cstdint>

#include "device_types.h"
#include "lbvh.h"

namespace rfwhip {

size_t sah_workspace_bytes(uint32_t n);

hipError_t sah_build(hipStream_t stream, const DevBox* boxes, uint32_t n, void* workspace, size_t workspace_bytes, Node4* nodes_out,
                     uint32_t* prim_order_out, uint32_t* node_count_out , int max_leaf, float trav_cost);

struct ForestTree { uint32_t first, count, node_base, pad; };
size_t sah_forest_workspace_bytes(uint32_t n, uint32_t n_trees);
hipError_t sah_build_forest(hipStream_t stream, const DevBox* boxes, uint32_t n, const ForestTree* trees, uint32_t n_trees, uint32_t largest_tree, void* workspace,
                            size_t workspace_bytes, Node4* nodes_base, uint32_t* prim_order_out, uint32_t* node_counts_out, int max_leaf, float trav_cost);
void launch_forest_relative_order(hipStream_t stream, uint32_t* order, uint32_t n, const ForestTree* trees, uint32_t n_trees);

void launch_refit_setup(hipStream_t s, const Node4* nodes, uint32_t n_nodes, uint32_t* parent_slot, uint32_t* n_internal);
void launch_refit(hipStream_t s, Node4* nodes, uint32_t n_nodes, const rfw_rt_triangle* tris, const uint32_t* order, const uint32_t* parent_slot,
                  const uint32_t* n_internal, uint32_t* arrive);

}
```

rfw-rs_amd/csrc/sah_build.hip:

```cpp
#include "sah_build.h"
#include "env_switches.h"

#include <hipcub/hipcub.hpp>

#include <chrono>
#include <cstdio>
#include <cstdlib>

namespace rfwhip {
namespace {

constexpr int kBlock = 256;
constexpr int kBins = 16;
constexpr uint32_t kSmall = 512;
constexpr uint32_t kSmallFew = 256;
inline uint32_t small_cap_for(uint32_t n) { return n <= 32768u ? kSmallFew : kSmall; }
constexpr uint32_t kNone = 0xffffffffu;
constexpr int kMaxLevels = 96;

struct SNode {
    uint32_t cb[6];
    uint32_t first, count;
    float lo[3];
    uint32_t left;
// ... 512 lines not shown
        for (uint32_t w = 0; w < wave; w++) { off[0] += s_cnt[j][w][0]; off[1] += s_cnt[j][w][1]; }
        if (in) {
            const unsigned long long m = right ? rm : lm;
            const uint32_t rank = __builtin_amdgcn_mbcnt_hi((uint32_t)(m >> 32), __builtin_amdgcn_mbcnt_lo((uint32_t)m, 0u));
            const uint32_t dest = (right ? first_r + off[1] : first_l + off[0]) + rank;
            order_out[dest] = order_in[p];
            nop_out[dest] = li + (right ? 1u : 0u);
            pbox_out[dest] = pbox_in[p];
        }
        for (int w = 0; w < kBlock / 64; w++) { run[0] += s_cnt[j][w][0]; run[1] += s_cnt[j][w][1]; }
    }
}

constexpr uint32_t kWaveRange = 64;
constexpr int kListCap = 96;

__device__ inline void wave_sync()
{
    __builtin_amdgcn_fence(__ATOMIC_ACQ_REL, "wavefront");
    __builtin_amdgcn_wave_barrier();
}

template <uint32_t CAP> struct SmallShared {
    static constexpr int kWaves = (int)(CAP / 64);
    float lo[3][CAP], hi[3][CAP];
    uint16_t perm[2][CAP];
    Bin bins[3 * kBins];
    Bin wbins[kWaves][3 * kBins];
    uint32_t cb[6];
    SplitChoice choice;
    SplitChoice wchoice[kWaves];
    uint32_t next_id;
    uint32_t wave_cnt[kWaves][2];
    uint32_t stack[3 * 12]; float stack_box[6 * 12];
    uint32_t list[3 * kListCap]; float list_box[6 * kListCap];
    uint32_t list_n, list_head;
    uint32_t wstack[kWaves][3 * 8]; float wstack_box[kWaves][6 * 8];
};

template <uint32_t CAP> __device__ inline void finish_range_wave(SmallShared<CAP>& S, const uint32_t wave, const uint32_t lane, uint32_t first, uint32_t count, uint32_t nid, float* nlo, float* nhi,
                                         const uint32_t gfirst, SNode* nodes, const int max_leaf, const float trav_cost)
{
    int sp = 0;
    for (;;) {
        if (count == 2u) {
            const uint32_t q0 = S.perm[0][first], q1 = S.perm[0][first + 1u];
            float l0[3], h0[3], l1[3], h1[3];
            bool sep = false, swap = false;
            for (int a = 0; a < 3; a++) {
                l0[a] = S.lo[a][q0]; h0[a] = S.hi[a][q0]; l1[a] = S.lo[a][q1]; h1[a] = S.hi[a][q1];
                const float c0 = 0.5f * (l0[a] + h0[a]), c1 = 0.5f * (l1[a] + h1[a]);
                if (!sep && c0 != c1) { sep = true; swap = c1 < c0; }
            }
            const float area = half_area(nlo, nhi);
            const bool split2 = (sep && half_area(l0, h0) + half_area(l1, h1) + trav_cost * area < 2.0f * area) || 2 > max_leaf;
            if (split2) {
                uint32_t li = 0;
                if (lane == 0) li = atomicAdd(&S.next_id, 2u);
                li = (uint32_t)__builtin_amdgcn_readfirstlane((int)li);
                if (lane == 0) {
                    SNode l, r;
                    init_child(l, gfirst + first, 1u, swap ? l1 : l0, swap ? h1 : h0, nid);
                    init_child(r, gfirst + first + 1u, 1u, swap ? l0 : l1, swap ? h0 : h1, nid);
                    nodes[li] = l;
                    nodes[li + 1] = r;
                    nodes[nid].left = li;
                    if (swap) { S.perm[0][first] = (uint16_t)q1; S.perm[0][first + 1u] = (uint16_t)q0; }
                }
                wave_sync();
            }
            if (sp == 0) break;
            sp--;
            first = S.wstack[wave][3 * sp + 0];
            count = S.wstack[wave][3 * sp + 1];
            nid = S.wstack[wave][3 * sp + 2];
            for (int a = 0; a < 3; a++) { nlo[a] = S.wstack_box[wave][6 * sp + a]; nhi[a] = S.wstack_box[wave][6 * sp + 3 + a]; }
            wave_sync();
            continue;
        }
        const bool mine = lane < count;
        const uint32_t q = mine ? S.perm[0][first + lane] : 0u;
        float cen[3] = {0.0f, 0.0f, 0.0f};
        int my_bin[3] = {0, 0, 0};
        bool split = false;
        int win = -1;
        SplitChoice s;
        if (count > 1) {
            if (lane < 3 * kBins) {
                Bin e; e.count = 0;
                for (int a = 0; a < 3; a++) { e.lo[a] = 0xffffffffu; e.hi[a] = 0u; }
                S.wbins[wave][lane] = e;
            }
            float clo[3], chi[3];
            for (int a = 0; a < 3; a++) {
                cen[a] = mine ? 0.5f * (S.lo[a][q] + S.hi[a][q]) : 0.0f;
                clo[a] = wave_min(mine ? cen[a] : INFINITY);
                chi[a] = wave_max(mine ? cen[a] : -INFINITY);
            }
            wave_sync();
            {
                float blo[3] = {0.0f, 0.0f, 0.0f}, bhi[3] = {0.0f, 0.0f, 0.0f};
                if (mine)
                    for (int a = 0; a < 3; a++) { my_bin[a] = bin_of(cen[a], clo[a], chi[a]); blo[a] = S.lo[a][q]; bhi[a] = S.hi[a][q]; }
                wave_add_to_bins(S.wbins[wave], mine, my_bin, blo, bhi);
            }
            wave_sync();
            win = sweep48(S.wbins[wave], lane, s);
            if ((int)lane == (win >= 0 ? win : 0)) S.wchoice[wave] = s;
            wave_sync();
            s = S.wchoice[wave];
            const float area = half_area(nlo, nhi);
            const float leaf_cost = (float)count * area;
            if (win >= 0 && (s.cost + trav_cost * area < leaf_cost || (int)count > max_leaf)) split = true;
            else if ((int)count > max_leaf) {
                split = true;
                win = -1;
                s.left_count = count / 2;
                for (int a = 0; a < 3; a++) { s.llo[a] = s.rlo[a] = nlo[a]; s.lhi[a] = s.rhi[a] = nhi[a]; }
            }
        }
        if (split) {
            const uint32_t lc = s.left_count, rc = count - lc;
            uint32_t li = 0;
            if (lane == 0) li = atomicAdd(&S.next_id, 2u);
            li = (uint32_t)__builtin_amdgcn_readfirstlane((int)li);
            if (lane == 0) {
                SNode l, r;
                init_child(l, gfirst + first, lc, s.llo, s.lhi, nid);
                init_child(r, gfirst + first + lc, rc, s.rlo, s.rhi, nid);
                nodes[li] = l;
                nodes[li + 1] = r;
                nodes[nid].left = li;
            }
            const bool left = mine && (win < 0 ? lane < lc : my_bin[s.axis] <= s.plane);
            const unsigned long long lm = __ballot(left), rm = __ballot(mine && !left);
            if (mine) {
                const unsigned long long m = left ? lm : rm;
                const uint32_t rank = __builtin_amdgcn_mbcnt_hi((uint32_t)(m >> 32), __builtin_amdgcn_mbcnt_lo((uint32_t)m, 0u));
                S.perm[1][first + (left ? rank : lc + rank)] = (uint16_t)q;
            }
            wave_sync();
            if (mine) S.perm[0][first + lane] = S.perm[1][first + lane];
            const bool left_next = lc <= rc;
            if (lane == 0) {
                S.wstack[wave][3 * sp + 0] = left_next ? first + lc : first;
                S.wstack[wave][3 * sp + 1] = left_next ? rc : lc;
                S.wstack[wave][3 * sp + 2] = left_next ? li + 1 : li;
                for (int a = 0; a < 3; a++) { S.wstack_box[wave][6 * sp + a] = left_next ? s.rlo[a] : s.llo[a]; S.wstack_box[wave][6 * sp + 3 + a] = left_next ? s.rhi[a] : s.lhi[a]; }
            }
            sp++;
            if (left_next) { count = lc; nid = li; for (int a = 0; a < 3; a++) { nlo[a] = s.llo[a]; nhi[a] = s.lhi[a]; } }
            else { first = first + lc; count = rc; nid = li + 1; for (int a = 0; a < 3; a++) { nlo[a] = s.rlo[a]; nhi[a] = s.rhi[a]; } }
            wave_sync();
            continue;
        }
        if (sp == 0) break;
        sp--;
        first = S.wstack[wave][3 * sp + 0];
        count = S.wstack[wave][3 * sp + 1];
        nid = S.wstack[wave][3 * sp + 2];
        for (int a = 0; a < 3; a++) { nlo[a] = S.wstack_box[wave][6 * sp + a]; nhi[a] = S.wstack_box[wave][6 * sp + 3 + a]; }
        wave_sync();
    }
}

template <uint32_t CAP> __global__ __launch_bounds__(CAP) void k_small(const DevBox* __restrict__ boxes, const uint32_t* __restrict__ order_in, uint32_t* order_out,
                                                 const uint32_t* __restrict__ small, Counters* ctr, SNode* nodes, int max_leaf, float trav_cost)
{
    __shared__ SmallShared<CAP> S;
    const uint32_t tid = threadIdx.x, lane = tid & 63u, wave = tid >> 6;
    if (blockIdx.x >= ctr->n_small) return;
    const uint32_t root = small[blockIdx.x];
    const uint32_t gfirst = nodes[root].first, gcount = nodes[root].count;
    if (tid < gcount) {
        const DevBox b = boxes[order_in[gfirst + tid]];
        for (int a = 0; a < 3; a++) { S.lo[a][tid] = b.lo[a]; S.hi[a][tid] = b.hi[a]; }
        S.perm[0][tid] = (uint16_t)tid;
    }
    if (tid == 0) {
        S.next_id = atomicAdd(&ctr->node_count, 2u * gcount);
        S.list_n = 0; S.list_head = 0;
        S.stack[0] = 0; S.stack[1] = gcount; S.stack[2] = root;
        for (int a = 0; a < 3; a++) { S.stack_box[a] = nodes[root].lo[a]; S.stack_box[3 + a] = nodes[root].hi[a]; }
    }
    __syncthreads();
    int sp = 1;
    while (sp > 0) {
        sp--;
        uint32_t first = S.stack[3 * sp + 0], count = S.stack[3 * sp + 1], nid = S.stack[3 * sp + 2];
        float nlo[3], nhi[3];
        for (int a = 0; a < 3; a++) { nlo[a] = S.stack_box[6 * sp + a]; nhi[a] = S.stack_box[6 * sp + 3 + a]; }
        __syncthreads();
        for (;;) {
            const bool list_full = S.list_n >= (uint32_t)kListCap;
            if (count <= kWaveRange && !list_full) {
                if ((int)count > max_leaf || count > 1) {
                    if (tid == 0) {
                        const uint32_t e = S.list_n++;
                        S.list[3 * e + 0] = first; S.list[3 * e + 1] = count; S.list[3 * e + 2] = nid;
                        for (int a = 0; a < 3; a++) { S.list_box[6 * e + a] = nlo[a]; S.list_box[6 * e + 3 + a] = nhi[a]; }
                    }
                    __syncthreads();
                }
                break;
            }
            if (count <= 1) break;
            if (tid < 6) S.cb[tid] = tid < 3 ? 0xffffffffu : 0u;
            if (tid < 3 * kBins) {
                Bin e; e.count = 0;
                for (int a = 0; a < 3; a++) { e.lo[a] = 0xffffffffu; e.hi[a] = 0u; }
                S.bins[tid] = e;
            }
            __syncthreads();
            const bool mine = tid < count;
            const uint32_t q = mine ? S.perm[0][first + tid] : 0u;
            float cen[3] = {0.0f, 0.0f, 0.0f};
            for (int a = 0; a < 3; a++) {
                cen[a] = mine ? 0.5f * (S.lo[a][q] + S.hi[a][q]) : 0.0f;
                const float l = wave_min(mine ? cen[a] : INFINITY), h = wave_max(mine ? cen[a] : -INFINITY);
                if (lane == 0 && l <= h) { atomicMin(&S.cb[a], f_order(l)); atomicMax(&S.cb[3 + a], f_order(h)); }
            }
            __syncthreads();
            int my_bin[3] = {0, 0, 0};
            {
                float blo[3] = {0.0f, 0.0f, 0.0f}, bhi[3] = {0.0f, 0.0f, 0.0f};
                if (mine)
                    for (int a = 0; a < 3; a++) { my_bin[a] = bin_of(cen[a], f_unorder(S.cb[a]), f_unorder(S.cb[3 + a])); blo[a] = S.lo[a][q]; bhi[a] = S.hi[a][q]; }
                wave_add_to_bins(S.bins, mine, my_bin, blo, bhi);
            }
            __syncthreads();
            if (wave == 0) {
                SplitChoice s;
                const int win = sweep48(S.bins, lane, s);
                if ((int)lane == (win >= 0 ? win : 0)) {
                    if (win < 0) s.axis = -1;
                    S.choice = s;
                }
            }
            __syncthreads();
            SplitChoice s = S.choice;
            bool split = false;
            {
                const float area = half_area(nlo, nhi);
                const float leaf_cost = (float)count * area;
                if (s.axis >= 0 && (s.cost + trav_cost * area < leaf_cost || (int)count > max_leaf)) split = true;
                else if ((int)count > max_leaf) {
                    split = true;
                    s.axis = -1;
                    s.left_count = count / 2;
                    for (int a = 0; a < 3; a++) { s.llo[a] = s.rlo[a] = nlo[a]; s.lhi[a] = s.rhi[a] = nhi[a]; }
                }
            }
            if (!split) break;
            const uint32_t lc = s.left_count, rc = count - lc, li = S.next_id;
            const bool left = mine && (s.axis < 0 ? tid < lc : my_bin[s.axis] <= s.plane);
            const unsigned long long lm = __ballot(left), rm = __ballot(mine && !left);
            if (lane == 0) { S.wave_cnt[wave][0] = (uint32_t)__popcll(lm); S.wave_cnt[wave][1] = (uint32_t)__popcll(rm); }
            __syncthreads();
            if (mine) {
                uint32_t off = 0;
                for (uint32_t w = 0; w < wave; w++) off += S.wave_cnt[w][left ? 0 : 1];
                const unsigned long long m = left ? lm : rm;
                const uint32_t rank = __builtin_amdgcn_mbcnt_hi((uint32_t)(m >> 32), __builtin_amdgcn_mbcnt_lo((uint32_t)m, 0u));
                S.perm[1][first + (left ? off + rank : lc + off + rank)] = (uint16_t)q;
            }
            if (tid == 0) {
                S.next_id = li + 2;
                SNode l, r;
                init_child(l, gfirst + first, lc, s.llo, s.lhi, nid);
                init_child(r, gfirst + first + lc, rc, s.rlo, s.rhi, nid);
                nodes[li] = l;
                nodes[li + 1] = r;
                nodes[nid].left = li;
                const bool left_next = lc <= rc;
                S.stack[3 * sp + 0] = left_next ? first + lc : first;
                S.stack[3 * sp + 1] = left_next ? rc : lc;
                S.stack[3 * sp + 2] = left_next ? li + 1 : li;
                for (int a = 0; a < 3; a++) { S.stack_box[6 * sp + a] = left_next ? s.rlo[a] : s.llo[a]; S.stack_box[6 * sp + 3 + a] = left_next ? s.rhi[a] : s.lhi[a]; }
            }
            __syncthreads();
            if (mine) S.perm[0][first + tid] = S.perm[1][first + tid];
            sp++;
            const bool left_next = lc <= rc;
            if (left_next) { count = lc; nid = li; for (int a = 0; a < 3; a++) { nlo[a] = s.llo[a]; nhi[a] = s.lhi[a]; } }
            else { first = first + lc; count = rc; nid = li + 1; for (int a = 0; a < 3; a++) { nlo[a] = s.rlo[a]; nhi[a] = s.rhi[a]; } }
            __syncthreads();
        }
    }
    __syncthreads();
    const uint32_t n_list = S.list_n;
    for (;;) {
        uint32_t e = 0;
        if (lane == 0) e = atomicAdd(&S.list_head, 1u);
        e = (uint32_t)__builtin_amdgcn_readfirstlane((int)e);
        if (e >= n_list) break;
        float nlo[3], nhi[3];
        for (int a = 0; a < 3; a++) { nlo[a] = S.list_box[6 * e + a]; nhi[a] = S.list_box[6 * e + 3 + a]; }
        finish_range_wave(S, wave, lane, S.list[3 * e + 0], S.list[3 * e + 1], S.list[3 * e + 2], nlo, nhi, gfirst, nodes, max_leaf, trav_cost);
    }
    __syncthreads();
    if (tid < gcount) order_out[gfirst + tid] = order_in[gfirst + S.perm[0][tid]];
}

__global__ void k_flag_nodes(uint32_t n_nodes_cap, const Counters* __restrict__ ctr, const SNode* __restrict__ nodes, uint32_t* flag4)
{
    const uint32_t i = blockIdx.x * kBlock + threadIdx.x;
    if (i >= n_nodes_cap) return;
    uint32_t f = 0;
    if (i < ctr->node_count && nodes[i].left != kNone) {
        uint32_t depth = 0, p = nodes[i].parent;
        while (p != kNone) { depth++; p = nodes[p].parent; }
        f = (depth & 1u) ? 0u : 1u;
    }
    flag4[i] = f;
}
__global__ void k_emit_nodes(uint32_t n_nodes_cap, const Counters* __restrict__ ctr, const SNode* __restrict__ nodes, const uint32_t* __restrict__ flag4,
                             const uint32_t* __restrict__ idx4, Node4* out_nodes, uint32_t* node_count_out)
{
    const uint32_t i = blockIdx.x * kBlock + threadIdx.x;
    if (i >= n_nodes_cap) return;
    const uint32_t total = ctr->node_count;
    if (i == 0) {
        if (nodes[0].left == kNone) {
            Node4 o;
            for (int k = 0; k < 4; k++) {
                o.lox[k] = o.loy[k] = o.loz[k] = INFINITY; o.hix[k] = o.hiy[k] = o.hiz[k] = -INFINITY;
                o.child[k] = kInvalidRef; o.pad[k] = 0;
            }
            if (nodes[0].count) {
                o.lox[0] = nodes[0].lo[0]; o.loy[0] = nodes[0].lo[1]; o.loz[0] = nodes[0].lo[2];
                o.hix[0] = nodes[0].hi[0]; o.hiy[0] = nodes[0].hi[1]; o.hiz[0] = nodes[0].hi[2];
                o.child[0] = make_leaf(nodes[0].first, nodes[0].count);
            }
            out_nodes[0] = o;
            if (node_count_out) *node_count_out = 1;
            return;
        }
        if (node_count_out) *node_count_out = idx4[total - 1] + flag4[total - 1];
    }
    if (i >= total || !flag4[i]) return;
    uint32_t kids[4];
    int nk = 0;
    for (uint32_t c = nodes[i].left; c < nodes[i].left + 2; c++) {
        if (nodes[c].left == kNone) kids[nk++] = c;
        else { kids[nk++] = nodes[c].left; kids[nk++] = nodes[c].left + 1; }
    }
    Node4 o;
    for (int k = 0; k < 4; k++) {
        if (k < nk) {
            const SNode& c = nodes[kids[k]];
            o.lox[k] = c.lo[0]; o.loy[k] = c.lo[1]; o.loz[k] = c.lo[2];
            o.hix[k] = c.hi[0]; o.hiy[k] = c.hi[1]; o.hiz[k] = c.hi[2];
            o.child[k] = c.left == kNone ? make_leaf(c.first, c.count) : idx4[kids[k]];
        } else {
            o.lox[k] = o.loy[k] = o.loz[k] = INFINITY; o.hix[k] = o.hiy[k] = o.hiz[k] = -INFINITY;
            o.child[k] = kInvalidRef;
        }
        o.pad[k] = 0;
    }
    out_nodes[idx4[i]] = o;
}

__global__ void k_forest_init(Counters* ctr, uint32_t n_trees)
{
    if (threadIdx.x == 0) { ctr->node_count = n_trees; ctr->n_active[0] = 0; ctr->n_active[1] = 0; ctr->n_small = 0; }
}
constexpr uint32_t kForestBoundsBlocks = 1024;
__device__ inline uint32_t tree_of_position(const ForestTree* __restrict__ trees, uint32_t n_trees, uint32_t i)
{
    uint32_t lo = 0, hi = n_trees;
    while (hi - lo > 1) {
        const uint32_t mid = (lo + hi) >> 1;
        if (trees[mid].first <= i) lo = mid; else hi = mid;
    }
    while (lo > 0 && trees[lo].count == 0) lo--;
    return lo;
}
__global__ __launch_bounds__(kBlock) void k_forest_bounds(const DevBox* __restrict__ boxes, const ForestTree* __restrict__ trees, uint32_t n_trees, uint32_t n, uint32_t chunk,
                                                         uint32_t* order, uint32_t* node_of_pos, uint32_t* bounds)
{
    const uint32_t begin = blockIdx.x * chunk, end = min(n, begin + chunk);
    float lo[3] = {INFINITY, INFINITY, INFINITY}, hi[3] = {-INFINITY, -INFINITY, -INFINITY};
    float clo[3] = {INFINITY, INFINITY, INFINITY}, chi[3] = {-INFINITY, -INFINITY, -INFINITY};
    uint32_t m = kNone, m_end = 0;
    auto flush = [&]() {
        uint32_t* b = bounds + (size_t)m * 12u;
        for (int a = 0; a < 3; a++) {
            atomicMin(&b[a], f_order(lo[a])); atomicMax(&b[3 + a], f_order(hi[a]));
            atomicMin(&b[6 + a], f_order(clo[a])); atomicMax(&b[9 + a], f_order(chi[a]));
            lo[a] = INFINITY; hi[a] = -INFINITY; clo[a] = INFINITY; chi[a] = -INFINITY;
        }
    };
    for (uint32_t i = begin + threadIdx.x; i < end; i += kBlock) {
        if (m == kNone || i >= m_end) {
            if (m != kNone) flush();
            m = tree_of_position(trees, n_trees, i);
            m_end = trees[m].first + trees[m].count;
        }
        order[i] = i;
        node_of_pos[i] = m;
        const DevBox bx = boxes[i];
        for (int a = 0; a < 3; a++) {
            const float l = bx.lo[a], h = bx.hi[a], c = 0.5f * (l + h);
            lo[a] = fminf(lo[a], l); hi[a] = fmaxf(hi[a], h);
            clo[a] = fminf(clo[a], c); chi[a] = fmaxf(chi[a], c);
        }
    }
    const unsigned long long have = __ballot(m != kNone);
    if (have == 0ull) return;
    const uint32_t lead_m = (uint32_t)__builtin_amdgcn_readlane((int)m, __ffsll((long long)have) - 1);
    if (__ballot(m != kNone && m != lead_m) == 0ull) {
        for (int a = 0; a < 3; a++) { lo[a] = wave_min(lo[a]); hi[a] = wave_max(hi[a]); clo[a] = wave_min(clo[a]); chi[a] = wave_max(chi[a]); }
        m = lead_m;
        if ((threadIdx.x & 63u) == 0u) flush();
    } else if (m != kNone) flush();
}
__global__ __launch_bounds__(64) void k_forest_roots(const ForestTree* __restrict__ trees, const uint32_t* __restrict__ bounds, Counters* ctr, SNode* nodes, uint32_t* active,
                                                    uint32_t* small, uint32_t* bin_slot, uint8_t* stamp, Bin* bins, uint32_t replicas, uint32_t small_cap)
{
    __shared__ uint32_t s_slot;
    const uint32_t m = blockIdx.x;
    const ForestTree t = trees[m];
    if (threadIdx.x == 0) {
        s_slot = kNone;
        const uint32_t* b = bounds + (size_t)m * 12u;
        SNode r;
        for (int a = 0; a < 3; a++) {
            r.lo[a] = f_unorder(b[a]); r.hi[a] = f_unorder(b[3 + a]);
            r.cb[a] = b[6 + a]; r.cb[3 + a] = b[9 + a];
        }
        r.first = t.first; r.count = t.count; r.left = kNone; r.parent = kNone;
        nodes[m] = r;
        if (t.count > small_cap) {
            const uint32_t slot = atomicAdd(&ctr->n_active[0], 1u);
            active[slot] = m; bin_slot[m] = slot; stamp[m] = 0;
            s_slot = slot;
        } else if (t.count) {
            small[atomicAdd(&ctr->n_small, 1u)] = m;
        }
    }
    __syncthreads();
    if (s_slot != kNone) {
        Bin e; e.count = 0;
        for (int a = 0; a < 3; a++) { e.lo[a] = 0xffffffffu; e.hi[a] = 0u; }
        for (uint32_t k = threadIdx.x; k < replicas * 3 * kBins; k += 64u) bins[(size_t)s_slot * replicas * 3 * kBins + k] = e;
    }
}
__global__ void k_forest_bounds_init(uint32_t* bounds, uint32_t n_words)
{
    const uint32_t i = blockIdx.x * kBlock + threadIdx.x;
    if (i < n_words) bounds[i] = (i % 6u) < 3u ? 0xffffffffu : 0u;
}
__global__ void k_flag_forest(uint32_t n_nodes_cap, const Counters* __restrict__ ctr, const SNode* __restrict__ nodes, uint32_t* flag4, uint32_t* tree_of)
{
    const uint32_t i = blockIdx.x * kBlock + threadIdx.x;
    if (i >= n_nodes_cap) return;
    uint32_t f = 0, root = kNone;
    if (i < ctr->node_count) {
        uint32_t depth = 0, r = i, p = nodes[i].parent;
        while (p != kNone) { depth++; r = p; p = nodes[p].parent; }
        root = r;
        if (nodes[i].left != kNone) f = (depth & 1u) ? 0u : 1u;
    }
    flag4[i] = f;
    tree_of[i] = root;
}
__global__ void k_index_forest(uint32_t n_nodes_cap, const Counters* __restrict__ ctr, const SNode* __restrict__ nodes, const uint32_t* __restrict__ flag4,
                               const uint32_t* __restrict__ tree_of, uint32_t* idx4, uint32_t* tree_nodes)
{
    const uint32_t i = blockIdx.x * kBlock + threadIdx.x;
    const bool wide = i < n_nodes_cap && i < ctr->node_count && flag4[i] != 0u;
    const bool is_root = wide && nodes[i].parent == kNone;
    if (is_root) idx4[i] = 0u;
    const uint32_t t = wide ? tree_of[i] : kNone;
    bool todo = wide && !is_root;
    while (__ballot(todo) != 0ull) {
        const unsigned long long pending = __ballot(todo);
        const uint32_t lead_tree = (uint32_t)__shfl((int)t, __ffsll((long long)pending) - 1);
        const unsigned long long mine = __ballot(todo && t == lead_tree);
        const uint32_t rank = __builtin_amdgcn_mbcnt_hi((uint32_t)(mine >> 32), __builtin_amdgcn_mbcnt_lo((uint32_t)mine, 0u));
        uint32_t base = 0;
        if (todo && t == lead_tree && rank == 0u) base = atomicAdd(&tree_nodes[lead_tree], (uint32_t)__popcll(mine));
        base = (uint32_t)__shfl((int)base, __ffsll((long long)mine) - 1);
        if (todo && t == lead_tree) { idx4[i] = 1u + base + rank; todo = false; }
    }
}
__global__ void k_emit_forest(uint32_t n_nodes_cap, uint32_t n_trees, const Counters* __restrict__ ctr, const SNode* __restrict__ nodes, const uint32_t* __restrict__ flag4,
                              const uint32_t* __restrict__ idx4, const uint32_t* __restrict__ tree_of, const ForestTree* __restrict__ trees,
                              const uint32_t* __restrict__ tree_nodes, Node4* out_base, uint32_t* node_counts_out)
{
    const uint32_t i = blockIdx.x * kBlock + threadIdx.x;
    if (i >= n_nodes_cap) return;
    const uint32_t total = ctr->node_count;
    if (i < n_trees) {
        if (nodes[i].left == kNone) {
            Node4 o;
            for (int k = 0; k < 4; k++) {
                o.lox[k] = o.loy[k] = o.loz[k] = INFINITY; o.hix[k] = o.hiy[k] = o.hiz[k] = -INFINITY;
                o.child[k] = kInvalidRef; o.pad[k] = 0;
            }
            if (nodes[i].count) {
                o.lox[0] = nodes[i].lo[0]; o.loy[0] = nodes[i].lo[1]; o.loz[0] = nodes[i].lo[2];
                o.hix[0] = nodes[i].hi[0]; o.hiy[0] = nodes[i].hi[1]; o.hiz[0] = nodes[i].hi[2];
                o.child[0] = make_leaf(0u, nodes[i].count);
            }
            out_base[trees[i].node_base] = o;
            if (node_counts_out) node_counts_out[i] = 1;
            return;
        }
        if (node_counts_out) node_counts_out[i] = tree_nodes[i] + 1u;
    }
    if (i >= total || !flag4[i]) return;
    const ForestTree t = trees[tree_of[i]];
    uint32_t kids[4];
    int nk = 0;
    for (uint32_t c = nodes[i].left; c < nodes[i].left + 2; c++) {
        if (nodes[c].left == kNone) kids[nk++] = c;
        else { kids[nk++] = nodes[c].left; kids[nk++] = nodes[c].left + 1; }
    }
    Node4 o;
    for (int k = 0; k < 4; k++) {
        if (k < nk) {
            const SNode& c = nodes[kids[k]];
            o.lox[k] = c.lo[0]; o.loy[k] = c.lo[1]; o.loz[k] = c.lo[2];
            o.hix[k] = c.hi[0]; o.hiy[k] = c.hi[1]; o.hiz[k] = c.hi[2];
            o.child[k] = c.left == kNone ? make_leaf(c.first - t.first, c.count) : idx4[kids[k]];
        } else {
            o.lox[k] = o.loy[k] = o.loz[k] = INFINITY; o.hix[k] = o.hiy[k] = o.hiz[k] = -INFINITY;
            o.child[k] = kInvalidRef;
        }
        o.pad[k] = 0;
    }
    out_base[t.node_base + idx4[i]] = o;
}
__global__ void k_forest_relative_order(uint32_t* order, uint32_t n, const ForestTree* __restrict__ trees, uint32_t n_trees)
{
    const uint32_t p = blockIdx.x * kBlock + threadIdx.x;
    if (p >= n) return;
    uint32_t lo = 0, hi = n_trees;
    while (hi - lo > 1) {
        const uint32_t mid = (lo + hi) / 2;
        if (trees[mid].first <= p) lo = mid; else hi = mid;
    }
    order[p] -= trees[lo].first;
}

__global__ void k_refit_setup(const Node4* __restrict__ nodes, uint32_t n_nodes, uint32_t* parent_slot, uint32_t* n_internal)
{
    const uint32_t i = blockIdx.x * kBlock + threadIdx.x;
    if (i >= n_nodes) return;
    if (i == 0) parent_slot[0] = kNone;
    uint32_t cnt = 0;
    for (uint32_t k = 0; k < 4; k++) {
        const uint32_t c = nodes[i].child[k];
        if (c == kInvalidRef || (c & kLeafBit)) continue;
        parent_slot[c] = 4u * i + k;
        cnt++;
    }
    n_internal[i] = cnt;
}

__global__ void k_refit_leaves(Node4* nodes, uint32_t n_nodes, const rfw_rt_triangle* __restrict__ tris, const uint32_t* __restrict__ order)
{
    const uint32_t t = blockIdx.x * kBlock + threadIdx.x;
    const uint32_t i = t >> 2, k = t & 3u;
    if (i >= n_nodes) return;
    const uint32_t c = nodes[i].child[k];
    if (c == kInvalidRef || !(c & kLeafBit)) return;
    const uint32_t first = c & kLeafFirstMask, count = ((c >> 27) & 15u) + 1u;
    float lo[3] = {INFINITY, INFINITY, INFINITY}, hi[3] = {-INFINITY, -INFINITY, -INFINITY};
    for (uint32_t j = 0; j < count; j++) {
        const float4* tp = reinterpret_cast<const float4*>(tris + order[first + j]);
        const float4 a = tp[0], b = tp[1], cc = tp[2];
        const float va[3] = {a.x, a.y, a.z}, vb[3] = {b.x, b.y, b.z}, vc[3] = {cc.x, cc.y, cc.z};
        for (int d = 0; d < 3; d++) {
            const float l = fminf(va[d], fminf(vb[d], vc[d])), h = fmaxf(va[d], fmaxf(vb[d], vc[d]));
            const float e = 1e-4f + 4e-6f * fmaxf(fabsf(l), fabsf(h));
            lo[d] = fminf(lo[d], l - e);
            hi[d] = fmaxf(hi[d], h + e);
        }
    }
    nodes[i].lox[k] = lo[0]; nodes[i].loy[k] = lo[1]; nodes[i].loz[k] = lo[2];
    nodes[i].hix[k] = hi[0]; nodes[i].hiy[k] = hi[1]; nodes[i].hiz[k] = hi[2];
}

__global__ void k_refit_up(Node4* nodes, uint32_t n_nodes, const uint32_t* __restrict__ parent_slot, const uint32_t* __restrict__ n_internal, uint32_t* arrive)
{
    uint32_t i = blockIdx.x * kBlock + threadIdx.x;
    if (i >= n_nodes || n_internal[i] != 0u) return;
    for (;;) {
        const uint32_t ps = parent_slot[i];
        if (ps == kNone) return;
        const volatile Node4* nd = nodes + i;
        float lo[3] = {INFINITY, INFINITY, INFINITY}, hi[3] = {-INFINITY, -INFINITY, -INFINITY};
        for (int k = 0; k < 4; k++) {
            if (nd->child[k] == kInvalidRef) continue;
            lo[0] = fminf(lo[0], nd->lox[k]); lo[1] = fminf(lo[1], nd->loy[k]); lo[2] = fminf(lo[2], nd->loz[k]);
            hi[0] = fmaxf(hi[0], nd->hix[k]); hi[1] = fmaxf(hi[1], nd->hiy[k]); hi[2] = fmaxf(hi[2], nd->hiz[k]);
        }
        const uint32_t p = ps >> 2, k = ps & 3u;
        nodes[p].lox[k] = lo[0]; nodes[p].loy[k] = lo[1]; nodes[p].loz[k] = lo[2];
        nodes[p].hix[k] = hi[0]; nodes[p].hiy[k] = hi[1]; nodes[p].hiz[k] = hi[2];
        __threadfence();
        asm volatile("s_waitcnt vmcnt(0)" ::: "memory");
        if (atomicAdd(&arrive[p], 1u) + 1u != n_internal[p]) return;
        __threadfence();
        i = p;
    }
}

struct Layout {
    size_t ctr, nodes, order[2], nop[2], pbox[2], active[2], small, bin_slot, stamp, splits, fill, bins[2], flag4, idx4, cub, total, cub_bytes;
    uint32_t node_cap, big_cap;
};
Layout make_layout(uint32_t n)
{
    Layout L{};
    size_t off = 0;
    auto take = [&](size_t bytes) { const size_t o = off; off = align_up(off + bytes, 256); return o; };
    const size_t m = n > 0 ? n : 1;
    L.node_cap = (uint32_t)(4 * m + 64);
    L.big_cap = (uint32_t)(2 * m / small_cap_for(n) + 2);
    L.ctr = take(sizeof(Counters));
    L.nodes = take((size_t)L.node_cap * sizeof(SNode));
    for (int k = 0; k < 2; k++) { L.order[k] = take(m * 4); L.nop[k] = take(m * 4); L.pbox[k] = take(m * sizeof(DevBox)); L.active[k] = take((size_t)L.big_cap * 4); }
    L.small = take((m + 1) * 4);
    L.bin_slot = take((size_t)L.node_cap * 4);
    L.stamp = take((size_t)L.node_cap);
    L.splits = take((size_t)L.node_cap * sizeof(Split));
    L.fill = take((size_t)L.node_cap * 4);
    for (int k = 0; k < 2; k++) L.bins[k] = take(((size_t)L.big_cap + 512) * 3 * kBins * sizeof(Bin));
    L.flag4 = take((size_t)L.node_cap * 4);
    L.idx4 = take((size_t)L.node_cap * 4);
    size_t cb = 0;
    (void)hipcub::DeviceScan::ExclusiveSum(nullptr, cb, (const uint32_t*)nullptr, (uint32_t*)nullptr, (int)L.node_cap);
    L.cub_bytes = cb + 256;
    L.cub = take(L.cub_bytes);
    L.total = off;
    return L;
}

inline uint32_t blocks(uint32_t n, uint32_t per = kBlock) { return (n + per - 1) / per; }

}

size_t sah_workspace_bytes(uint32_t n) { return make_layout(n).total; }

hipError_t sah_build(hipStream_t s, const DevBox* boxes, uint32_t n, void* workspace, size_t workspace_bytes, Node4* nodes_out, uint32_t* order_out,
                     uint32_t* node_count_out, int max_leaf, float trav_cost)
{
    const Layout L = make_layout(n);
    if (L.total > workspace_bytes) return hipErrorInvalidValue;
    max_leaf = max_leaf < 1 ? 1 : (max_leaf > kMaxLeafTris ? kMaxLeafTris : max_leaf);
    char* w = static_cast<char*>(workspace);
    Counters* ctr = (Counters*)(w + L.ctr);
    SNode* nodes = (SNode*)(w + L.nodes);
    uint32_t* order[2] = {(uint32_t*)(w + L.order[0]), (uint32_t*)(w + L.order[1])};
    uint32_t* nop[2] = {(uint32_t*)(w + L.nop[0]), (uint32_t*)(w + L.nop[1])};
    uint32_t* active[2] = {(uint32_t*)(w + L.active[0]), (uint32_t*)(w + L.active[1])};
    uint32_t* small = (uint32_t*)(w + L.small);
    uint32_t* bin_slot = (uint32_t*)(w + L.bin_slot);
    uint8_t* stamp = (uint8_t*)(w + L.stamp);
    DevBox* pbox[2] = {(DevBox*)(w + L.pbox[0]), (DevBox*)(w + L.pbox[1])};
    Split* splits = (Split*)(w + L.splits);
    uint32_t* fill = (uint32_t*)(w + L.fill);
    Bin* bins[2] = {(Bin*)(w + L.bins[0]), (Bin*)(w + L.bins[1])};
    uint32_t* flag4 = (uint32_t*)(w + L.flag4);
    uint32_t* idx4 = (uint32_t*)(w + L.idx4);

    {
        hipError_t me = hipMemsetAsync(nodes, 0xff, (size_t)L.node_cap * sizeof(SNode), s);
        if (me == hipSuccess) me = hipMemsetAsync(stamp, 0xff, (size_t)L.node_cap, s);
        if (me != hipSuccess) return me;
    }
    hipLaunchKernelGGL(k_root_init, dim3(1), dim3(64), 0, s, ctr);
    if (n) hipLaunchKernelGGL(k_root_bounds, dim3(std::min(blocks(n), 1024u)), dim3(kBlock), 0, s, boxes, n, ctr, order[0], nop[0]);
    const uint32_t small_cap = small_cap_for(n);
    auto level_ub = [&](int l) { return (uint32_t)std::min<uint64_t>(l < 31 ? (1ull << l) : (1ull << 31), (uint64_t)n / small_cap + 1); };
    const uint32_t bin_groups = blocks(n);
    auto level_replicas = [&](int l) { return std::max(1u, std::min(32u, bin_groups / (8u * level_ub(l)))); };
    hipLaunchKernelGGL(k_root_node, dim3(1), dim3(64), 0, s, n, ctr, nodes, active[0], small, bin_slot, stamp, bins[0], level_replicas(0), small_cap);
    const bool dbg = env_switches().build_trace;
    auto now = [] { return std::chrono::steady_clock::now(); };
    auto msf = [](auto a, auto b) { return std::chrono::duration<float, std::milli>(b - a).count(); };
    if (dbg) (void)hipStreamSynchronize(s);
    const auto t_start = now();
    int cur = 0, level = 0;
    auto run_level = [&]() {
        const uint32_t par = (uint32_t)(level & 1);
        const uint32_t ub = level_ub(level), reps = level_replicas(level), reps_next = level_replicas(level + 1);
        const DevBox* pin = level == 0 ? boxes : pbox[cur];
        hipLaunchKernelGGL(k_bin, dim3(bin_groups), dim3(kBlock), 0, s, pin, nop[cur], nodes, bin_slot, stamp, bins[par], n, ctr, (uint32_t)level, reps);
        hipLaunchKernelGGL(k_split, dim3(blocks(ub, kBlock / 64)), dim3(kBlock), 0, s, active[par], active[par ^ 1], (uint32_t)level, ctr, nodes, bins[par], bins[par ^ 1], bin_slot, stamp, splits, fill,
                           small, reps, reps_next, small_cap);
        if (ub * 64u <= blocks(n))
            hipLaunchKernelGGL(k_partition_chunk, dim3(blocks(n, kPartChunk * kBlock)), dim3(kBlock), 0, s, pin, pbox[cur ^ 1], order[cur], nop[cur], order[cur ^ 1], nop[cur ^ 1],
                               nodes, splits, stamp, fill, n, (uint32_t)level);
        else
            hipLaunchKernelGGL(k_partition, dim3(blocks(n)), dim3(kBlock), 0, s, pin, pbox[cur ^ 1], order[cur], nop[cur], order[cur ^ 1], nop[cur ^ 1], nodes, splits, stamp, fill, n,
                               (uint32_t)level);
        cur ^= 1;
        level++;
    };
    uint32_t counts[4] = {0, 0, 0, 0};
    auto read_counts = [&]() -> hipError_t {
        hipError_t e = hipMemcpyAsync(counts, ctr, sizeof(counts), hipMemcpyDeviceToHost, s);
        if (e == hipSuccess) e = hipStreamSynchronize(s);
        return e;
    };
    if (n > small_cap) {
        int expect = n > 65536u ? 8 : 2;
        for (uint32_t v = n / small_cap; v > 1; v >>= 1) expect++;
        while (level < expect && level < kMaxLevels) run_level();
    }
    hipError_t e = read_counts();
    if (e != hipSuccess) return e;
    while (counts[1 + (level & 1)] > 0 && level < kMaxLevels) {
        if (counts[1 + (level & 1)] > L.big_cap) return hipErrorInvalidValue;
        for (int k = 0; k < 4 && level < kMaxLevels; k++) run_level();
        if ((e = read_counts()) != hipSuccess) return e;
    }
    const auto t_p1 = now();
    if (counts[1 + (level & 1)] > 0) return hipErrorInvalidValue;
    const uint32_t n_small = counts[3];
    if (n_small && small_cap == kSmall) hipLaunchKernelGGL(HIP_KERNEL_NAME(k_small<kSmall>), dim3(n_small), dim3(kSmall), 0, s, boxes, order[cur], order_out, small, ctr, nodes, max_leaf, trav_cost);
    else if (n_small) hipLaunchKernelGGL(HIP_KERNEL_NAME(k_small<kSmallFew>), dim3(n_small), dim3(kSmallFew), 0, s, boxes, order[cur], order_out, small, ctr, nodes, max_leaf, trav_cost);
    if (dbg) { (void)hipStreamSynchronize(s); fprintf(stderr, "sah n=%u: phase1 %.3f ms (%d levels), phase2 %.3f ms (%u small ranges)\n", n, msf(t_start, t_p1), level, msf(t_p1, now()), n_small); }
    hipLaunchKernelGGL(k_flag_nodes, dim3(blocks(L.node_cap)), dim3(kBlock), 0, s, L.node_cap, ctr, nodes, flag4);
    size_t cub_bytes = L.cub_bytes;
    e = hipcub::DeviceScan::ExclusiveSum(w + L.cub, cub_bytes, flag4, idx4, (int)L.node_cap, s);
    if (e != hipSuccess) return e;
    hipLaunchKernelGGL(k_emit_nodes, dim3(blocks(L.node_cap)), dim3(kBlock), 0, s, L.node_cap, ctr, nodes, flag4, idx4, nodes_out, node_count_out);
    return hipGetLastError();
}

size_t sah_forest_workspace_bytes(uint32_t n, uint32_t n_trees)
{
    return make_layout(n + n_trees).total + align_up((size_t)(4 * ((size_t)n + n_trees) + 64 + n_trees) * 4, 256) + align_up((size_t)n_trees * 4, 256) +
           align_up((size_t)n_trees * 12 * 4, 256);
}

hipError_t sah_build_forest(hipStream_t s, const DevBox* boxes, uint32_t n, const ForestTree* trees, uint32_t n_trees, uint32_t largest_tree, void* workspace,
                            size_t workspace_bytes, Node4* nodes_base, uint32_t* order_out, uint32_t* node_counts_out, int max_leaf, float trav_cost)
{
    if (n == 0 || n_trees == 0) return hipErrorInvalidValue;
    const Layout L = make_layout(n + n_trees);
    const size_t tree_of_off = L.total, tree_nodes_off = tree_of_off + align_up((size_t)L.node_cap * 4, 256);
    if (sah_forest_workspace_bytes(n, n_trees) > workspace_bytes) return hipErrorInvalidValue;
    max_leaf = max_leaf < 1 ? 1 : (max_leaf > kMaxLeafTris ? kMaxLeafTris : max_leaf);
    char* w = static_cast<char*>(workspace);
    Counters* ctr = (Counters*)(w + L.ctr);
    SNode* nodes = (SNode*)(w + L.nodes);
    uint32_t* order[2] = {(uint32_t*)(w + L.order[0]), (uint32_t*)(w + L.order[1])};
    uint32_t* nop[2] = {(uint32_t*)(w + L.nop[0]), (uint32_t*)(w + L.nop[1])};
    uint32_t* active[2] = {(uint32_t*)(w + L.active[0]), (uint32_t*)(w + L.active[1])};
    uint32_t* small = (uint32_t*)(w + L.small);
    uint32_t* bin_slot = (uint32_t*)(w + L.bin_slot);
    uint8_t* stamp = (uint8_t*)(w + L.stamp);
    DevBox* pbox[2] = {(DevBox*)(w + L.pbox[0]), (DevBox*)(w + L.pbox[1])};
    Split* splits = (Split*)(w + L.splits);
    uint32_t* fill = (uint32_t*)(w + L.fill);
    Bin* bins[2] = {(Bin*)(w + L.bins[0]), (Bin*)(w + L.bins[1])};
    uint32_t* flag4 = (uint32_t*)(w + L.flag4);
    uint32_t* idx4 = (uint32_t*)(w + L.idx4);
    uint32_t* tree_of = (uint32_t*)(w + tree_of_off);
    uint32_t* tree_nodes = (uint32_t*)(w + tree_nodes_off);
    uint32_t* tree_bounds = (uint32_t*)(w + tree_nodes_off + align_up((size_t)n_trees * 4, 256));
    hipError_t e = hipMemsetAsync(nodes, 0xff, (size_t)L.node_cap * sizeof(SNode), s);
    if (e == hipSuccess) e = hipMemsetAsync(stamp, 0xff, (size_t)L.node_cap, s);
    if (e == hipSuccess) e = hipMemsetAsync(tree_nodes, 0, (size_t)n_trees * 4, s);
    if (e != hipSuccess) return e;
    const uint32_t small_cap = small_cap_for(n);
    auto level_ub = [&](int l) { return (uint32_t)std::min<uint64_t>(l < 20 ? ((uint64_t)n_trees << l) : ~0ull >> 1, (uint64_t)n / small_cap + 1); };
    const uint32_t bin_groups = blocks(n);
    auto level_replicas = [&](int l) { return std::max(1u, std::min(32u, bin_groups / (8u * level_ub(l)))); };
    hipLaunchKernelGGL(k_forest_init, dim3(1), dim3(64), 0, s, ctr, n_trees);
    hipLaunchKernelGGL(k_forest_bounds_init, dim3(blocks(n_trees * 12u)), dim3(kBlock), 0, s, tree_bounds, n_trees * 12u);
    {
        const uint32_t chunk = (uint32_t)align_up(((size_t)n + kForestBoundsBlocks - 1) / kForestBoundsBlocks, kBlock);
        hipLaunchKernelGGL(k_forest_bounds, dim3(blocks(n, chunk)), dim3(kBlock), 0, s, boxes, trees, n_trees, n, chunk, order[0], nop[0], tree_bounds);
    }
    hipLaunchKernelGGL(k_forest_roots, dim3(n_trees), dim3(64), 0, s, trees, tree_bounds, ctr, nodes, active[0], small, bin_slot, stamp, bins[0], level_replicas(0), small_cap);
    int cur = 0, level = 0;
    auto run_level = [&]() {
        const uint32_t par = (uint32_t)(level & 1);
        const uint32_t ub = level_ub(level), reps = level_replicas(level), reps_next = level_replicas(level + 1);
        const DevBox* pin = level == 0 ? boxes : pbox[cur];
        hipLaunchKernelGGL(k_bin, dim3(bin_groups), dim3(kBlock), 0, s, pin, nop[cur], nodes, bin_slot, stamp, bins[par], n, ctr, (uint32_t)level, reps);
        hipLaunchKernelGGL(k_split, dim3(blocks(ub, kBlock / 64)), dim3(kBlock), 0, s, active[par], active[par ^ 1], (uint32_t)level, ctr, nodes, bins[par], bins[par ^ 1], bin_slot, stamp, splits, fill,
                           small, reps, reps_next, small_cap);
        if ((largest_tree >> std::min(level, 31)) >= 64u * kBlock)
            hipLaunchKernelGGL(k_partition_chunk, dim3(blocks(n, kPartChunk * kBlock)), dim3(kBlock), 0, s, pin, pbox[cur ^ 1], order[cur], nop[cur], order[cur ^ 1], nop[cur ^ 1],
                               nodes, splits, stamp, fill, n, (uint32_t)level);
        else
            hipLaunchKernelGGL(k_partition, dim3(blocks(n)), dim3(kBlock), 0, s, pin, pbox[cur ^ 1], order[cur], nop[cur], order[cur ^ 1], nop[cur ^ 1], nodes, splits, stamp, fill, n,
                               (uint32_t)level);
        cur ^= 1;
        level++;
    };
    uint32_t counts[4] = {0, 0, 0, 0};
    auto read_counts = [&]() -> hipError_t {
        hipError_t e2 = hipMemcpyAsync(counts, ctr, sizeof(counts), hipMemcpyDeviceToHost, s);
        if (e2 == hipSuccess) e2 = hipStreamSynchronize(s);
        return e2;
    };
    if (largest_tree > small_cap) {
        int expect = largest_tree > 65536u ? 8 : 3;
        for (uint32_t v = largest_tree / small_cap; v > 1; v >>= 1) expect++;
        while (level < expect && level < kMaxLevels) run_level();
    }
    if ((e = read_counts()) != hipSuccess) return e;
    while (counts[1 + (level & 1)] > 0 && level < kMaxLevels) {
        if (counts[1 + (level & 1)] > L.big_cap) return hipErrorInvalidValue;
        for (int k = 0; k < 4 && level < kMaxLevels; k++) run_level();
        if ((e = read_counts()) != hipSuccess) return e;
    }
    if (counts[1 + (level & 1)] > 0) return hipErrorInvalidValue;
    const uint32_t n_small = counts[3];
    if (n_small && small_cap == kSmall) hipLaunchKernelGGL(HIP_KERNEL_NAME(k_small<kSmall>), dim3(n_small), dim3(kSmall), 0, s, boxes, order[cur], order_out, small, ctr, nodes, max_leaf, trav_cost);
    else if (n_small) hipLaunchKernelGGL(HIP_KERNEL_NAME(k_small<kSmallFew>), dim3(n_small), dim3(kSmallFew), 0, s, boxes, order[cur], order_out, small, ctr, nodes, max_leaf, trav_cost);
    hipLaunchKernelGGL(k_flag_forest, dim3(blocks(L.node_cap)), dim3(kBlock), 0, s, L.node_cap, ctr, nodes, flag4, tree_of);
    hipLaunchKernelGGL(k_index_forest, dim3(blocks(L.node_cap)), dim3(kBlock), 0, s, L.node_cap, ctr, nodes, flag4, tree_of, idx4, tree_nodes);
    hipLaunchKernelGGL(k_emit_forest, dim3(blocks(L.node_cap)), dim3(kBlock), 0, s, L.node_cap, n_trees, ctr, nodes, flag4, idx4, tree_of, trees, tree_nodes, nodes_base, node_counts_out);
    return hipGetLastError();
}
void launch_forest_relative_order(hipStream_t s, uint32_t* order, uint32_t n, const ForestTree* trees, uint32_t n_trees)
{
    if (n && n_trees) hipLaunchKernelGGL(k_forest_relative_order, dim3(blocks(n)), dim3(kBlock), 0, s, order, n, trees, n_trees);
}

void launch_refit_setup(hipStream_t s, const Node4* nodes, uint32_t n_nodes, uint32_t* parent_slot, uint32_t* n_internal)
{
    if (n_nodes) hipLaunchKernelGGL(k_refit_setup, dim3(blocks(n_nodes)), dim3(kBlock), 0, s, nodes, n_nodes, parent_slot, n_internal);
}
void launch_refit(hipStream_t s, Node4* nodes, uint32_t n_nodes, const rfw_rt_triangle* tris, const uint32_t* order, const uint32_t* parent_slot,
                  const uint32_t* n_internal, uint32_t* arrive)
{
    if (!n_nodes) return;
    (void)hipMemsetAsync(arrive, 0, (size_t)n_nodes * 4, s);
    hipLaunchKernelGGL(k_refit_leaves, dim3(blocks(4 * n_nodes)), dim3(kBlock), 0, s, nodes, n_nodes, tris, order);
    hipLaunchKernelGGL(k_refit_up, dim3(blocks(n_nodes)), dim3(kBlock), 0, s, nodes, n_nodes, parent_slot, n_internal, arrive);
}

}
```

Before: 8439.

## Add cost-optimal SAH collapse of binary BVH into BVH4 on host and GPU

Replaces the fixed even-depth (GPU) and greedy largest-area (host) binary-to-4-wide collapse with a dynamic-programming collapse. It computes per-node cost tables bottom-up over subtree slot budgets and picks which binary nodes become wide nodes. The GPU path adds a bottom-up atomic-arrival kernel to build the tables, and the flag and emit kernels now walk those tables. The aim is a lower expected traversal cost in the resulting BVH4 at the price of extra build work and workspace. The collapse option defaults to the SAH mode.

```diff
diff --git a/rfw-rs_amd/csrc/api_frame.cpp b/rfw-rs_amd/csrc/api_frame.cpp
--- a/rfw-rs_amd/csrc/api_frame.cpp
+++ b/rfw-rs_amd/csrc/api_frame.cpp
@@ -1063,6 +1063,15 @@
     else if (k == "sky_b") I->sky[2] = (float)value;
     else if (k == "sah_max_leaf") I->sah_max_leaf = std::max(1, std::min((int)value, kMaxLeafTris));
     else if (k == "sah_trav_cost") I->sah_trav_cost = (float)value;
+    else if (k == "collapse") {
+        if (value != 0.0 && value != 1.0) return fail(I, RFW_HIP_E_INVALID, "set_option: collapse is 0 (even depth) or 1 (cost-optimal)");
+        if ((int)value != I->collapse) {
+            I->collapse = (int)value;
+            for (auto& kv : I->meshes) kv.second.dirty = true;
+            I->meshes_dirty = true;
+            I->layout_valid = false;
+        }
+    }
     else if (k == "spatial_splits") I->split_tau = (float)std::max(0.0, value);
     else if (k == "stream_run") {
         const uint32_t r = (uint32_t)value;
diff --git a/rfw-rs_amd/csrc/api_internal.h b/rfw-rs_amd/csrc/api_internal.h
--- a/rfw-rs_amd/csrc/api_internal.h
+++ b/rfw-rs_amd/csrc/api_internal.h
@@ -238,6 +238,7 @@
     int build_threads = 8;
     int sah_max_leaf = 8;
     float sah_trav_cost = 1.0f;
+    int collapse = kCollapseSah;
 
     std::map<uint32_t, MeshHost> meshes;
     std::map<uint32_t, InstList> inst_lists;
diff --git a/rfw-rs_amd/csrc/api_scene.cpp b/rfw-rs_amd/csrc/api_scene.cpp
--- a/rfw-rs_amd/csrc/api_scene.cpp
+++ b/rfw-rs_amd/csrc/api_scene.cpp
@@ -72,7 +72,7 @@
         for (int a = 0; a < 3; a++) { boxes[sp.index].lo[a] = sp.lo[a]; boxes[sp.index].hi[a] = sp.hi[a]; }
         pad_box(boxes[sp.index]);
     }
-    build_bvh4_host(boxes, I->sah_max_leaf, I->build_threads, m.bvh, I->sah_trav_cost);
+    build_bvh4_host(boxes, I->sah_max_leaf, I->build_threads, m.bvh, I->sah_trav_cost, I->collapse ? kHostCollapseSah : kHostCollapseGreedy);
     m.packets.resize(n);
     for (size_t k = 0; k < n; k++) {
         const uint32_t id = m.bvh.prim_order[k];
@@ -234,7 +234,7 @@
 {
     if (sah) {
         HIP_TRY(I, sah_ws.ensure(sah_workspace_bytes(n)));
-        const hipError_t se = sah_build(s, boxes, n, sah_ws.ptr, sah_ws.cap, raw, order, count, I->sah_max_leaf, I->sah_trav_cost);
+        const hipError_t se = sah_build(s, boxes, n, sah_ws.ptr, sah_ws.cap, raw, order, count, I->sah_max_leaf, I->sah_trav_cost, I->collapse);
         if (se != hipErrorInvalidValue) { HIP_TRY(I, se); return RFW_HIP_OK; }
     }
     HIP_TRY(I, lbvh_build(s, boxes, n, lbvh_ws.ptr, lbvh_ws.cap, raw, order, count));
@@ -285,7 +285,7 @@
                     const MeshRecord& r = I->mesh_records[q];
                     record_boxes(I, L.s, q, plan.from_heads, L.boxes.ptr);
                     const hipError_t e = sah_build(L.s, L.boxes.ptr, r.tri_count, L.ws.ptr, L.ws.cap, I->d_blas_raw.ptr + r.node_base, I->d_blas_order.ptr + r.tri_base,
-                                                   I->d_mesh_node_counts.ptr + q, I->sah_max_leaf, I->sah_trav_cost);
+                                                   I->d_mesh_node_counts.ptr + q, I->sah_max_leaf, I->sah_trav_cost, I->collapse);
                     if (e == hipErrorInvalidValue) { redo[q] = 1; continue; }
                     if (e != hipSuccess) { lane_err[k] = e; return; }
                     record_finish(I, L.s, q, plan);
@@ -428,7 +428,7 @@
         else launch_triangle_boxes(I->stream, I->d_triangles.ptr, L.static_tris, I->d_tri_boxes.ptr);
         for (size_t q = 0; q < n_static; q++) patch_boxes(I, I->stream, (uint32_t)q, I->d_tri_boxes.ptr + I->mesh_records[q].tri_base);
         const hipError_t fe = sah_build_forest(I->stream, I->d_tri_boxes.ptr, L.static_tris, I->d_forest.ptr, (uint32_t)n_static, L.max_n, I->d_sah_ws.ptr, I->d_sah_ws.cap,
-                                               I->d_blas_raw.ptr, I->d_blas_order.ptr, I->d_mesh_node_counts.ptr, I->sah_max_leaf, I->sah_trav_cost);
+                                               I->d_blas_raw.ptr, I->d_blas_order.ptr, I->d_mesh_node_counts.ptr, I->sah_max_leaf, I->sah_trav_cost, I->collapse);
         if (fe == hipSuccess) {
             if (from_heads) HIP_TRY(I, hipStreamWaitEvent(I->stream, I->ev_records, 0));
             launch_make_packets(I->stream, I->d_triangles.ptr, I->d_blas_order.ptr, L.static_tris, 0u, I->d_packets.ptr);
diff --git a/rfw-rs_amd/csrc/bvh_host.cpp b/rfw-rs_amd/csrc/bvh_host.cpp
--- a/rfw-rs_amd/csrc/bvh_host.cpp
+++ b/rfw-rs_amd/csrc/bvh_host.cpp
@@ -163,9 +163,60 @@
     return n;
 }
 
-}
-
-void build_bvh4_host(const std::vector<PrimBox>& boxes, int max_leaf, int threads, HostBvh4& out, float trav_cost)
+struct CostTab { float c[3] = {0.0f, 0.0f, 0.0f}; uint32_t pick = 0; };
+inline uint32_t settle(uint32_t pick, uint32_t j)
+{
+    if (j >= 3u && (pick & 32u)) return 3u;
+    if (j >= 2u && (pick & 16u)) return 2u;
+    return 1u;
+}
+inline uint32_t left_share(uint32_t pick, uint32_t s) { return s == 4u ? (pick >> 2) & 3u : (s == 3u ? pick & 3u : 1u); }
+std::vector<CostTab> collapse_tables(const std::vector<Node2>& n2, uint32_t used)
+{
+    std::vector<CostTab> tab(used);
+    for (uint32_t i = used; i-- > 0;) {
+        if (n2[i].count > 0 || n2[i].left == 0) continue;
+        const float* cl = tab[n2[i].left].c;
+        const float* cr = tab[n2[i].right].c;
+        CostTab& t = tab[i];
+        const float d2 = cl[0] + cr[0];
+        float d3 = cl[0] + cr[1], d4 = cl[0] + cr[2], v;
+        uint32_t k3 = 1u, k4 = 1u;
+        v = cl[1] + cr[0]; if (v < d3) { d3 = v; k3 = 2u; }
+        v = cl[1] + cr[1]; if (v < d4) { d4 = v; k4 = 2u; }
+        v = cl[2] + cr[0]; if (v < d4) { d4 = v; k4 = 3u; }
+        t.c[0] = d4 + n2[i].box.half_area();
+        const bool open2 = d2 < t.c[0];
+        t.c[1] = open2 ? d2 : t.c[0];
+        const bool open3 = d3 < t.c[1];
+        t.c[2] = open3 ? d3 : t.c[1];
+        t.pick = k3 | (k4 << 2) | (open2 ? 16u : 0u) | (open3 ? 32u : 0u);
+    }
+    return tab;
+}
+int cost_children(const std::vector<Node2>& n2, const std::vector<CostTab>& tab, uint32_t w, uint32_t* kids)
+{
+    struct E { uint32_t node, j; };
+    E st[4];
+    int sp = 0, nk = 0;
+    const uint32_t ls = left_share(tab[w].pick, 4u);
+    st[sp++] = {n2[w].right, 4u - ls};
+    st[sp++] = {n2[w].left, ls};
+    while (sp > 0 && nk < 4) {
+        const E e = st[--sp];
+        const Node2& c = n2[e.node];
+        const uint32_t s = c.count > 0 ? 1u : settle(tab[e.node].pick, e.j);
+        if (s == 1u) { kids[nk++] = e.node; continue; }
+        const uint32_t l = left_share(tab[e.node].pick, s);
+        st[sp++] = {c.right, s - l};
+        st[sp++] = {c.left, l};
+    }
+    return nk;
+}
+
+}
+
+void build_bvh4_host(const std::vector<PrimBox>& boxes, int max_leaf, int threads, HostBvh4& out, float trav_cost, int collapse)
 {
     out.nodes.clear();
     out.prim_order.clear();
@@ -183,6 +234,8 @@
         set_child(out.nodes[0], 0, n2[0].box, make_leaf(n2[0].first, n2[0].count));
         return;
     }
+    std::vector<CostTab> tab;
+    if (collapse == kHostCollapseSah) tab = collapse_tables(n2, b2.next_node.load());
     struct Work { uint32_t n4, n2; };
     std::vector<Work> stack;
     stack.push_back({0u, 0u});
@@ -191,7 +244,15 @@
         stack.pop_back();
         uint32_t kids[4] = {n2[w.n2].left, n2[w.n2].right, 0, 0};
         int nk = 2;
-        while (nk < 4) {
+        if (collapse == kHostCollapseSah) nk = cost_children(n2, tab, w.n2, kids);
+        else if (collapse == kHostCollapseEvenDepth) {
+            nk = 0;
+            for (const uint32_t c : {n2[w.n2].left, n2[w.n2].right}) {
+                if (n2[c].count > 0) kids[nk++] = c;
+                else { kids[nk++] = n2[c].left; kids[nk++] = n2[c].right; }
+            }
+        }
+        while (collapse == kHostCollapseGreedy && nk < 4) {
             int best = -1;
             float best_area = -1.0f;
             for (int i = 0; i < nk; i++) {
diff --git a/rfw-rs_amd/csrc/bvh_host.h b/rfw-rs_amd/csrc/bvh_host.h
--- a/rfw-rs_amd/csrc/bvh_host.h
+++ b/rfw-rs_amd/csrc/bvh_host.h
@@ -15,7 +15,8 @@
     std::vector<uint32_t> prim_order;
 };
 
-void build_bvh4_host(const std::vector<PrimBox>& boxes, int max_leaf, int threads, HostBvh4& out, float trav_cost = 1.0f);
+enum { kHostCollapseGreedy = 0, kHostCollapseSah = 1, kHostCollapseEvenDepth = 2 };
+void build_bvh4_host(const std::vector<PrimBox>& boxes, int max_leaf, int threads, HostBvh4& out, float trav_cost = 1.0f, int collapse = kHostCollapseGreedy);
 
 uint64_t validate_bvh4(const HostBvh4& bvh, const std::vector<PrimBox>& boxes);
 
diff --git a/rfw-rs_amd/csrc/sah_build.h b/rfw-rs_amd/csrc/sah_build.h
--- a/rfw-rs_amd/csrc/sah_build.h
+++ b/rfw-rs_amd/csrc/sah_build.h
@@ -9,15 +9,18 @@
 
 namespace rfwhip {
 
+enum { kCollapseEvenDepth = 0, kCollapseSah = 1 };
+
 size_t sah_workspace_bytes(uint32_t n);
 
 hipError_t sah_build(hipStream_t stream, const DevBox* boxes, uint32_t n, void* workspace, size_t workspace_bytes, Node4* nodes_out,
-                     uint32_t* prim_order_out, uint32_t* node_count_out , int max_leaf, float trav_cost);
+                     uint32_t* prim_order_out, uint32_t* node_count_out , int max_leaf, float trav_cost, int collapse = kCollapseEvenDepth);
 
 struct ForestTree { uint32_t first, count, node_base, pad; };
 size_t sah_forest_workspace_bytes(uint32_t n, uint32_t n_trees);
 hipError_t sah_build_forest(hipStream_t stream, const DevBox* boxes, uint32_t n, const ForestTree* trees, uint32_t n_trees, uint32_t largest_tree, void* workspace,
-                            size_t workspace_bytes, Node4* nodes_base, uint32_t* prim_order_out, uint32_t* node_counts_out, int max_leaf, float trav_cost);
+                            size_t workspace_bytes, Node4* nodes_base, uint32_t* prim_order_out, uint32_t* node_counts_out, int max_leaf, float trav_cost,
+                            int collapse = kCollapseEvenDepth);
 void launch_forest_relative_order(hipStream_t stream, uint32_t* order, uint32_t n, const ForestTree* trees, uint32_t n_trees);
 
 void launch_refit_setup(hipStream_t s, const Node4* nodes, uint32_t n_nodes, uint32_t* parent_slot, uint32_t* n_internal);
diff --git a/rfw-rs_amd/csrc/sah_build.hip b/rfw-rs_amd/csrc/sah_build.hip
--- a/rfw-rs_amd/csrc/sah_build.hip
+++ b/rfw-rs_amd/csrc/sah_build.hip
@@ -838,19 +838,128 @@
     if (tid < gcount) order_out[gfirst + tid] = order_in[gfirst + S.perm[0][tid]];
 }
 
-__global__ void k_flag_nodes(uint32_t n_nodes_cap, const Counters* __restrict__ ctr, const SNode* __restrict__ nodes, uint32_t* flag4)
+struct CTab {
+    float c[3];
+    uint32_t pick;
+};
+__host__ __device__ inline uint32_t settle(uint32_t pick, uint32_t j)
+{
+    if (j >= 3u && (pick & 32u)) return 3u;
+    if (j >= 2u && (pick & 16u)) return 2u;
+    return 1u;
+}
+__host__ __device__ inline uint32_t left_share(uint32_t pick, uint32_t s) { return s == 4u ? (pick >> 2) & 3u : (s == 3u ? pick & 3u : 1u); }
+__host__ __device__ inline uint32_t child_slots(uint32_t pick, uint32_t j, bool is_left)
+{
+    uint32_t s = settle(pick, j);
+    if (s == 1u) s = 4u;
+    const uint32_t ls = left_share(pick, s);
+    return is_left ? ls : s - ls;
+}
+__host__ __device__ inline CTab collapse_costs(const float* cl, const float* cr, float area)
+{
+    CTab t;
+    const float d2 = cl[0] + cr[0];
+    float d3 = cl[0] + cr[1], d4 = cl[0] + cr[2], v;
+    uint32_t k3 = 1u, k4 = 1u;
+    v = cl[1] + cr[0]; if (v < d3) { d3 = v; k3 = 2u; }
+    v = cl[1] + cr[1]; if (v < d4) { d4 = v; k4 = 2u; }
+    v = cl[2] + cr[0]; if (v < d4) { d4 = v; k4 = 3u; }
+    t.c[0] = d4 + area;
+    const bool open2 = d2 < t.c[0];
+    t.c[1] = open2 ? d2 : t.c[0];
+    const bool open3 = d3 < t.c[1];
+    t.c[2] = open3 ? d3 : t.c[1];
+    t.pick = k3 | (k4 << 2) | (open2 ? 16u : 0u) | (open3 ? 32u : 0u);
+    return t;
+}
+__global__ void k_collapse_costs(uint32_t n_nodes_cap, const Counters* __restrict__ ctr, const SNode* __restrict__ nodes, CTab* tab, uint32_t* arrive)
+{
+    const uint32_t i = blockIdx.x * kBlock + threadIdx.x;
+    if (i >= n_nodes_cap || i >= ctr->node_count || nodes[i].left != kNone) return;
+    uint32_t me = i, p = nodes[i].parent;
+    float mine[3] = {0.0f, 0.0f, 0.0f};
+    while (p != kNone) {
+        if (atomicAdd(&arrive[p], 1u) == 0u) return;
+        const uint32_t l = nodes[p].left, sib = me == l ? l + 1u : l;
+        float other[3] = {0.0f, 0.0f, 0.0f};
+        if (nodes[sib].left != kNone)
+            for (int j = 0; j < 3; j++) other[j] = __hip_atomic_load(&tab[sib].c[j], __ATOMIC_RELAXED, __HIP_MEMORY_SCOPE_AGENT);
+        const CTab t = collapse_costs(me == l ? mine : other, me == l ? other : mine, half_area(nodes[p].lo, nodes[p].hi));
+        for (int j = 0; j < 3; j++) { __hip_atomic_store(&tab[p].c[j], t.c[j], __ATOMIC_RELAXED, __HIP_MEMORY_SCOPE_AGENT); mine[j] = t.c[j]; }
+        tab[p].pick = t.pick;
+        asm volatile("s_waitcnt vmcnt(0)" ::: "memory");
+        me = p;
+        p = nodes[p].parent;
+    }
+}
+__device__ inline uint32_t slots_of(const SNode* __restrict__ nodes, const CTab* __restrict__ tab, uint32_t i, const bool want_root, uint32_t* root)
+{
+    uint32_t g1 = 1u, g2 = 2u, g3 = 3u, c = i, p = nodes[i].parent, res = 0u;
+    bool known = p == kNone;
+    while (p != kNone) {
+        const uint32_t pick = tab[p].pick, up = nodes[p].parent;
+        const bool is_left = nodes[p].left == c;
+        if (!known) {
+            if (up == kNone) { const uint32_t a = child_slots(pick, 1u, is_left); res = a == 1u ? g1 : (a == 2u ? g2 : g3); known = true; }
+            else {
+                const uint32_t a1 = child_slots(pick, 1u, is_left), a2 = child_slots(pick, 2u, is_left), a3 = child_slots(pick, 3u, is_left);
+                const uint32_t n1 = a1 == 1u ? g1 : (a1 == 2u ? g2 : g3), n2 = a2 == 1u ? g1 : (a2 == 2u ? g2 : g3), n3 = a3 == 1u ? g1 : (a3 == 2u ? g2 : g3);
+                g1 = n1; g2 = n2; g3 = n3;
+                if (g1 == g2 && g2 == g3) { res = g1; known = true; }
+            }
+        }
+        if (known && !want_root) break;
+        c = p; p = up;
+    }
+    if (root) *root = c;
+    return res;
+}
+__host__ __device__ inline bool is_wide(uint32_t pick, uint32_t slots) { return slots == 0u || settle(pick, slots) == 1u; }
+__device__ inline int wide_children(const SNode* __restrict__ nodes, const CTab* __restrict__ tab, uint32_t i, uint32_t* kids)
+{
+    int nk = 0;
+    if (!tab) {
+        for (uint32_t c = nodes[i].left; c < nodes[i].left + 2; c++) {
+            if (nodes[c].left == kNone) kids[nk++] = c;
+            else { kids[nk++] = nodes[c].left; kids[nk++] = nodes[c].left + 1; }
+        }
+        return nk;
+    }
+    uint32_t st_node[4], st_j[4];
+    int sp = 0;
+    {
+        const uint32_t l = nodes[i].left, ls = left_share(tab[i].pick, 4u);
+        st_node[sp] = l + 1u; st_j[sp++] = 4u - ls;
+        st_node[sp] = l; st_j[sp++] = ls;
+    }
+    while (sp > 0 && nk < 4) {
+        sp--;
+        const uint32_t c = st_node[sp], j = st_j[sp], l = nodes[c].left;
+        const uint32_t pick = l == kNone ? 0u : tab[c].pick, s = settle(pick, j);
+        if (l == kNone || s == 1u) { kids[nk++] = c; continue; }
+        const uint32_t ls = left_share(pick, s);
+        st_node[sp] = l + 1u; st_j[sp++] = s - ls;
+        st_node[sp] = l; st_j[sp++] = ls;
+    }
+    return nk;
+}
+__global__ void k_flag_nodes(uint32_t n_nodes_cap, const Counters* __restrict__ ctr, const SNode* __restrict__ nodes, const CTab* __restrict__ tab, uint32_t* flag4)
 {
     const uint32_t i = blockIdx.x * kBlock + threadIdx.x;
     if (i >= n_nodes_cap) return;
     uint32_t f = 0;
     if (i < ctr->node_count && nodes[i].left != kNone) {
-        uint32_t depth = 0, p = nodes[i].parent;
-        while (p != kNone) { depth++; p = nodes[p].parent; }
-        f = (depth & 1u) ? 0u : 1u;
+        if (tab) f = is_wide(tab[i].pick, slots_of(nodes, tab, i, false, nullptr)) ? 1u : 0u;
+        else {
+            uint32_t depth = 0, p = nodes[i].parent;
+            while (p != kNone) { depth++; p = nodes[p].parent; }
+            f = (depth & 1u) ? 0u : 1u;
+        }
     }
     flag4[i] = f;
 }
-__global__ void k_emit_nodes(uint32_t n_nodes_cap, const Counters* __restrict__ ctr, const SNode* __restrict__ nodes, const uint32_t* __restrict__ flag4,
+__global__ void k_emit_nodes(uint32_t n_nodes_cap, const Counters* __restrict__ ctr, const SNode* __restrict__ nodes, const CTab* __restrict__ tab, const uint32_t* __restrict__ flag4,
                              const uint32_t* __restrict__ idx4, Node4* out_nodes, uint32_t* node_count_out)
 {
     const uint32_t i = blockIdx.x * kBlock + threadIdx.x;
@@ -876,11 +985,7 @@
     }
     if (i >= total || !flag4[i]) return;
     uint32_t kids[4];
-    int nk = 0;
-    for (uint32_t c = nodes[i].left; c < nodes[i].left + 2; c++) {
-        if (nodes[c].left == kNone) kids[nk++] = c;
-        else { kids[nk++] = nodes[c].left; kids[nk++] = nodes[c].left + 1; }
-    }
+    const int nk = wide_children(nodes, tab, i, kids);
     Node4 o;
     for (int k = 0; k < 4; k++) {
         if (k < nk) {
@@ -987,12 +1092,15 @@
     const uint32_t i = blockIdx.x * kBlock + threadIdx.x;
     if (i < n_words) bounds[i] = (i % 6u) < 3u ? 0xffffffffu : 0u;
 }
-__global__ void k_flag_forest(uint32_t n_nodes_cap, const Counters* __restrict__ ctr, const SNode* __restrict__ nodes, uint32_t* flag4, uint32_t* tree_of)
+__global__ void k_flag_forest(uint32_t n_nodes_cap, const Counters* __restrict__ ctr, const SNode* __restrict__ nodes, const CTab* __restrict__ tab, uint32_t* flag4, uint32_t* tree_of)
 {
     const uint32_t i = blockIdx.x * kBlock + threadIdx.x;
     if (i >= n_nodes_cap) return;
     uint32_t f = 0, root = kNone;
-    if (i < ctr->node_count) {
+    if (i < ctr->node_count && tab) {
+        const uint32_t slots = slots_of(nodes, tab, i, true, &root);
+        if (nodes[i].left != kNone) f = is_wide(tab[i].pick, slots) ? 1u : 0u;
+    } else if (i < ctr->node_count) {
         uint32_t depth = 0, r = i, p = nodes[i].parent;
         while (p != kNone) { depth++; r = p; p = nodes[p].parent; }
         root = r;
@@ -1021,7 +1129,7 @@
         if (todo && t == lead_tree) { idx4[i] = 1u + base + rank; todo = false; }
     }
 }
-__global__ void k_emit_forest(uint32_t n_nodes_cap, uint32_t n_trees, const Counters* __restrict__ ctr, const SNode* __restrict__ nodes, const uint32_t* __restrict__ flag4,
+__global__ void k_emit_forest(uint32_t n_nodes_cap, uint32_t n_trees, const Counters* __restrict__ ctr, const SNode* __restrict__ nodes, const CTab* __restrict__ tab, const uint32_t* __restrict__ flag4,
                               const uint32_t* __restrict__ idx4, const uint32_t* __restrict__ tree_of, const ForestTree* __restrict__ trees,
                               const uint32_t* __restrict__ tree_nodes, Node4* out_base, uint32_t* node_counts_out)
 {
@@ -1049,11 +1157,7 @@
     if (i >= total || !flag4[i]) return;
     const ForestTree t = trees[tree_of[i]];
     uint32_t kids[4];
-    int nk = 0;
-    for (uint32_t c = nodes[i].left; c < nodes[i].left + 2; c++) {
-        if (nodes[c].left == kNone) kids[nk++] = c;
-        else { kids[nk++] = nodes[c].left; kids[nk++] = nodes[c].left + 1; }
-    }
+    const int nk = wide_children(nodes, tab, i, kids);
     Node4 o;
     for (int k = 0; k < 4; k++) {
         if (k < nk) {
@@ -1146,7 +1250,7 @@
 }
 
 struct Layout {
-    size_t ctr, nodes, order[2], nop[2], pbox[2], active[2], small, bin_slot, stamp, splits, fill, bins[2], flag4, idx4, cub, total, cub_bytes;
+    size_t ctr, nodes, order[2], nop[2], pbox[2], active[2], small, bin_slot, stamp, splits, fill, bins[2], flag4, idx4, ctab, arrive, cub, total, cub_bytes;
     uint32_t node_cap, big_cap;
 };
 Layout make_layout(uint32_t n)
@@ -1168,6 +1272,8 @@
     for (int k = 0; k < 2; k++) L.bins[k] = take(((size_t)L.big_cap + 512) * 3 * kBins * sizeof(Bin));
     L.flag4 = take((size_t)L.node_cap * 4);
     L.idx4 = take((size_t)L.node_cap * 4);
+    L.ctab = take((size_t)L.node_cap * sizeof(CTab));
+    L.arrive = take((size_t)L.node_cap * 4);
     size_t cb = 0;
     (void)hipcub::DeviceScan::ExclusiveSum(nullptr, cb, (const uint32_t*)nullptr, (uint32_t*)nullptr, (int)L.node_cap);
     L.cub_bytes = cb + 256;
@@ -1183,7 +1289,7 @@
 size_t sah_workspace_bytes(uint32_t n) { return make_layout(n).total; }
 
 hipError_t sah_build(hipStream_t s, const DevBox* boxes, uint32_t n, void* workspace, size_t workspace_bytes, Node4* nodes_out, uint32_t* order_out,
-                     uint32_t* node_count_out, int max_leaf, float trav_cost)
+                     uint32_t* node_count_out, int max_leaf, float trav_cost, int collapse)
 {
     const Layout L = make_layout(n);
     if (L.total > workspace_bytes) return hipErrorInvalidValue;
@@ -1203,6 +1309,8 @@
     Bin* bins[2] = {(Bin*)(w + L.bins[0]), (Bin*)(w + L.bins[1])};
     uint32_t* flag4 = (uint32_t*)(w + L.flag4);
     uint32_t* idx4 = (uint32_t*)(w + L.idx4);
+    CTab* ctab = collapse == kCollapseSah ? (CTab*)(w + L.ctab) : nullptr;
+    uint32_t* arrive = (uint32_t*)(w + L.arrive);
 
     {
         hipError_t me = hipMemsetAsync(nodes, 0xff, (size_t)L.node_cap * sizeof(SNode), s);
@@ -1262,11 +1370,15 @@
     if (n_small && small_cap == kSmall) hipLaunchKernelGGL(HIP_KERNEL_NAME(k_small<kSmall>), dim3(n_small), dim3(kSmall), 0, s, boxes, order[cur], order_out, small, ctr, nodes, max_leaf, trav_cost);
     else if (n_small) hipLaunchKernelGGL(HIP_KERNEL_NAME(k_small<kSmallFew>), dim3(n_small), dim3(kSmallFew), 0, s, boxes, order[cur], order_out, small, ctr, nodes, max_leaf, trav_cost);
     if (dbg) { (void)hipStreamSynchronize(s); fprintf(stderr, "sah n=%u: phase1 %.3f ms (%d levels), phase2 %.3f ms (%u small ranges)\n", n, msf(t_start, t_p1), level, msf(t_p1, now()), n_small); }
-    hipLaunchKernelGGL(k_flag_nodes, dim3(blocks(L.node_cap)), dim3(kBlock), 0, s, L.node_cap, ctr, nodes, flag4);
+    if (ctab) {
+        if ((e = hipMemsetAsync(arrive, 0, (size_t)L.node_cap * 4, s)) != hipSuccess) return e;
+        hipLaunchKernelGGL(k_collapse_costs, dim3(blocks(L.node_cap)), dim3(kBlock), 0, s, L.node_cap, ctr, nodes, ctab, arrive);
+    }
+    hipLaunchKernelGGL(k_flag_nodes, dim3(blocks(L.node_cap)), dim3(kBlock), 0, s, L.node_cap, ctr, nodes, ctab, flag4);
     size_t cub_bytes = L.cub_bytes;
     e = hipcub::DeviceScan::ExclusiveSum(w + L.cub, cub_bytes, flag4, idx4, (int)L.node_cap, s);
     if (e != hipSuccess) return e;
-    hipLaunchKernelGGL(k_emit_nodes, dim3(blocks(L.node_cap)), dim3(kBlock), 0, s, L.node_cap, ctr, nodes, flag4, idx4, nodes_out, node_count_out);
+    hipLaunchKernelGGL(k_emit_nodes, dim3(blocks(L.node_cap)), dim3(kBlock), 0, s, L.node_cap, ctr, nodes, ctab, flag4, idx4, nodes_out, node_count_out);
     return hipGetLastError();
 }
 
@@ -1277,7 +1389,7 @@
 }
 
 hipError_t sah_build_forest(hipStream_t s, const DevBox* boxes, uint32_t n, const ForestTree* trees, uint32_t n_trees, uint32_t largest_tree, void* workspace,
-                            size_t workspace_bytes, Node4* nodes_base, uint32_t* order_out, uint32_t* node_counts_out, int max_leaf, float trav_cost)
+                            size_t workspace_bytes, Node4* nodes_base, uint32_t* order_out, uint32_t* node_counts_out, int max_leaf, float trav_cost, int collapse)
 {
     if (n == 0 || n_trees == 0) return hipErrorInvalidValue;
     const Layout L = make_layout(n + n_trees);
@@ -1299,6 +1411,8 @@
     Bin* bins[2] = {(Bin*)(w + L.bins[0]), (Bin*)(w + L.bins[1])};
     uint32_t* flag4 = (uint32_t*)(w + L.flag4);
     uint32_t* idx4 = (uint32_t*)(w + L.idx4);
+    CTab* ctab = collapse == kCollapseSah ? (CTab*)(w + L.ctab) : nullptr;
+    uint32_t* arrive = (uint32_t*)(w + L.arrive);
     uint32_t* tree_of = (uint32_t*)(w + tree_of_off);
     uint32_t* tree_nodes = (uint32_t*)(w + tree_nodes_off);
     uint32_t* tree_bounds = (uint32_t*)(w + tree_nodes_off + align_up((size_t)n_trees * 4, 256));
@@ -1355,9 +1469,13 @@
     const uint32_t n_small = counts[3];
     if (n_small && small_cap == kSmall) hipLaunchKernelGGL(HIP_KERNEL_NAME(k_small<kSmall>), dim3(n_small), dim3(kSmall), 0, s, boxes, order[cur], order_out, small, ctr, nodes, max_leaf, trav_cost);
     else if (n_small) hipLaunchKernelGGL(HIP_KERNEL_NAME(k_small<kSmallFew>), dim3(n_small), dim3(kSmallFew), 0, s, boxes, order[cur], order_out, small, ctr, nodes, max_leaf, trav_cost);
-    hipLaunchKernelGGL(k_flag_forest, dim3(blocks(L.node_cap)), dim3(kBlock), 0, s, L.node_cap, ctr, nodes, flag4, tree_of);
+    if (ctab) {
+        if ((e = hipMemsetAsync(arrive, 0, (size_t)L.node_cap * 4, s)) != hipSuccess) return e;
+        hipLaunchKernelGGL(k_collapse_costs, dim3(blocks(L.node_cap)), dim3(kBlock), 0, s, L.node_cap, ctr, nodes, ctab, arrive);
+    }
+    hipLaunchKernelGGL(k_flag_forest, dim3(blocks(L.node_cap)), dim3(kBlock), 0, s, L.node_cap, ctr, nodes, ctab, flag4, tree_of);
     hipLaunchKernelGGL(k_index_forest, dim3(blocks(L.node_cap)), dim3(kBlock), 0, s, L.node_cap, ctr, nodes, flag4, tree_of, idx4, tree_nodes);
-    hipLaunchKernelGGL(k_emit_forest, dim3(blocks(L.node_cap)), dim3(kBlock), 0, s, L.node_cap, n_trees, ctr, nodes, flag4, idx4, tree_of, trees, tree_nodes, nodes_base, node_counts_out);
+    hipLaunchKernelGGL(k_emit_forest, dim3(blocks(L.node_cap)), dim3(kBlock), 0, s, L.node_cap, n_trees, ctr, nodes, ctab, flag4, idx4, tree_of, trees, tree_nodes, nodes_base, node_counts_out);
     return hipGetLastError();
 }
 void launch_forest_relative_order(hipStream_t s, uint32_t* order, uint32_t n, const ForestTree* trees, uint32_t n_trees)
```

Result: no change. 8585 (median of 6 runs) (+1.7%).
